# OpenRobotLab/EmbodiedScan

Measured on AMD Instinct MI355X. Metric: scans/sec (train step) mv-3ddet, 20x(480x640) RGB-D views, higher is better.
Workload: dtype bf16; 1 GPU; mv-3ddet ResNet-50(w16) + MinkResNet34 + FCAF3DHeadRotMat, 20 views 480x640, 100k points/scan, bf16 matrix cores with f32 accumulate / f32 master weights, full train step incl. H2D of the batch and AdamW; views=20, parallelism=dp1, h2d=157 MB per step as ONE copy from a pinned slab on a copy stream, double-buffered

## Files before the change

### embodiedscan_amd/csrc/halo.hip

```cpp
#include "common.h"
#include "../../include/es_hip.h"
#include <type_traits>

typedef float f32x4 __attribute__((ext_vector_type(4)));
typedef __bf16 bf16x8_t __attribute__((ext_vector_type(8)));
#ifdef ES_EMU
#define ES_SCHED_FENCE() ((void)0)
#define ES_UNIFORM(x) (x)
#define ES_WAIT_LGKM0() ((void)0)
#else
#define ES_WAIT_LGKM0() __builtin_amdgcn_s_waitcnt(0xC07F)
#define ES_SCHED_FENCE() __builtin_amdgcn_sched_barrier(0)
#define ES_UNIFORM(x) __builtin_amdgcn_readfirstlane(x)
#endif

#define HL_BM 256
#define HL_K 27
#define HL_UMAX 704
#define HL_HT 8192

__device__ __attribute__((aligned(16))) unsigned short g_hl_zero[8];

__global__ __launch_bounds__(512) void k_halo_plan(const int* __restrict__ nbr, int n_out, int K,
                                                   unsigned short* __restrict__ loc, int* __restrict__ hrows,
                                                   int* __restrict__ hcnt) {
  constexpr int NE = HL_BM * HL_K;
  __shared__ __attribute__((aligned(16))) int nb[NE];
  __shared__ unsigned short slotOf[NE];
  __shared__ int hk[HL_HT];
  __shared__ unsigned short hv[HL_HT];
  __shared__ int cnt;
  const int t = threadIdx.x, tile = blockIdx.x;
  const long long e0 = (long long)tile * NE, eN = (long long)n_out * K;
  for (int i = t; i < HL_HT; i += 512) hk[i] = -1;
  if (t == 0) cnt = 0;
  for (int i = t; i < NE / 4; i += 512) {
    int4 v = make_int4(-1, -1, -1, -1);
    const long long e = e0 + (long long)i * 4;
    if (e + 3 < eN) v = *(const int4*)(nbr + e);
    else {
      if (e < eN) v.x = nbr[e];
      if (e + 1 < eN) v.y = nbr[e + 1];
      if (e + 2 < eN) v.z = nbr[e + 2];
    }
    ((int4*)nb)[i] = v;
  }
  __syncthreads();
  for (int e = t; e < NE; e += 512) {
    const int v = nb[e];
    unsigned short so = 0xFFFFu;
    if (v >= 0) {
      unsigned s = ((unsigned)v * 2654435761u) >> (32 - 13);
      for (;;) {
        const int old = atomicCAS(&hk[s], -1, v);
        if (old == -1 || old == v) break;
        s = (s + 1) & (HL_HT - 1);
      }
      so = (unsigned short)s;
    }
    slotOf[e] = so;
  }
  __syncthreads();
  int* const list = nb;
  for (int sl = t; sl < HL_HT; sl += 512) {
    const int v = hk[sl];
    const unsigned long long m = __ballot(v >= 0);
    int base = 0;
    if ((t & 63) == 0 && m) base = atomicAdd(&cnt, __popcll(m));
    base = __shfl(base, 0, 64);
    if (v >= 0) {
      const int pos = base + __popcll(m & ((1ull << (t & 63)) - 1ull));
      list[pos] = v;
      hv[sl] = (unsigned short)pos;
    }
  }
  __syncthreads();
  const int nU = cnt;
  unsigned short* const rk = (unsigned short*)hk;
  int* const hr = hrows + (size_t)tile * NE;
  for (int i = t; i < nU; i += 512) {
    const int v = list[i];
    int r = 0;
    for (int j = 0; j < nU; ++j) r += list[j] < v ? 1 : 0;
    rk[i] = (unsigned short)r;
    hr[r] = v;
  }
  if (t == 0) hcnt[tile] = nU;
  __syncthreads();
  unsigned int* const dst = (unsigned int*)(loc + (size_t)tile * NE);
  for (int i = t; i < NE / 2; i += 512) {
    const unsigned int s0 = slotOf[2 * i], s1 = slotOf[2 * i + 1];
    const unsigned int p0 = s0 == 0xFFFFu ? 0xFFFFu : rk[hv[s0]], p1 = s1 == 0xFFFFu ? 0xFFFFu : rk[hv[s1]];
    dst[i] = p0 | (p1 << 16);
  }
}

extern "C" size_t es_halo_plan_rows(int n_out) { return (size_t)es_cdiv(n_out, HL_BM) * HL_BM; }

extern "C" int es_halo_plan(const int* nbr, int n_out, int K, void* loc, int* hrows, int* hcnt, void* stream) {
  if (n_out <= 0) return 0;
  if (K != HL_K || nbr == nullptr) return -4;
  hipLaunchKernelGGL(k_halo_plan, dim3(es_cdiv(n_out, HL_BM)), dim3(512), 0, (hipStream_t)stream, nbr, n_out, K,
                     (unsigned short*)loc, hrows, hcnt);
  ES_CHECK_LAUNCH();
  return 0;
}

struct HlSeq { int ti, pg, c, tap; };

template <int BNT>
__global__ __launch_bounds__(512, 2) void k_spconv_halo(const unsigned short* __restrict__ Xh, int ldx,
                                                        const unsigned short* __restrict__ W, int Kd, int N,
                                                        const unsigned short* __restrict__ loc, const int* __restrict__ hrows,
                                                        const int* __restrict__ hcnt, int n_out, const float* __restrict__ bias,
                                                        float* __restrict__ Y, int ldy, int accumulate, int colTiles, int total,
                                                        int per, int mirror) {
  constexpr int RB = 128;
  constexpr int ZROW = HL_UMAX;
  constexpr int H_BYTES = (HL_UMAX + 1) * RB;
  constexpr int B_BYTES = BNT * RB;
  constexpr int OFF_B = H_BYTES, OFF_LOC = OFF_B + 3 * B_BYTES, OFF_TAP = OFF_LOC + HL_BM * HL_K * 2;
  constexpr int NH = HL_UMAX * 8 / 512;
  constexpr int NB = BNT / 64;
  constexpr int NF = BNT / 32;
  __shared__ __attribute__((aligned(16))) unsigned char smem[OFF_TAP + 64 * 4];
  unsigned short* const locS = (unsigned short*)(smem + OFF_LOC);
  int* const tapS = (int*)(smem + OFF_TAP);
  const int t = threadIdx.x, lane = t & 63, wv = t >> 6;
  const int wr = wv >> 1, wc = wv & 1;
  for (int it = 0;; ++it) {
  const int lx = (int)(blockIdx.x >> 3) + it * (int)(gridDim.x >> 3);
  const int L = (int)(blockIdx.x & 7) * per + lx;
  if (lx >= per || L >= total) break;
  if (it > 0) __syncthreads();
  const int rt = L / colTiles, ct = L - rt * colTiles;
  const int row0 = rt * HL_BM, n0 = ct * BNT;
  const int nU = hcnt[rt];
  const int nP = nU > HL_UMAX ? (nU + HL_UMAX - 1) / HL_UMAX : 1;
  const int* const hr = hrows + (size_t)rt * HL_BM * HL_K;

  if (t < 32) tapS[t] = 0;
  if (t < 32) ((unsigned int*)(smem + ZROW * RB))[t] = 0u;
  __syncthreads();
  {
    const uint4* g = (const uint4*)(loc + (size_t)row0 * HL_K);
    for (int i = t; i < HL_BM * HL_K / 8; i += 512) {
      const uint4 v = g[i];
      ((uint4*)locS)[i] = v;
      const unsigned int w4[4] = {v.x, v.y, v.z, v.w};
#pragma unroll
      for (int q = 0; q < 8; ++q) {
        const unsigned int p = (w4[q >> 1] >> ((q & 1) * 16)) & 0xFFFFu;
        if (p != 0xFFFFu) tapS[mirror ? HL_K - 1 - (i * 8 + q) % HL_K : (i * 8 + q) % HL_K] = 1;
      }
    }
  }
  __syncthreads();
  unsigned int tm = 0;
  {
    const int f = (lane < HL_K) ? tapS[lane] : 0;
    tm = ES_UNIFORM((unsigned int)__ballot(f));
  }
  const int nT = __popc(tm);

  f32x4 acc[4][NF];
#pragma unroll
  for (int a = 0; a < 4; ++a)
#pragma unroll
    for (int b = 0; b < NF; ++b) acc[a][b] = (f32x4){0.f, 0.f, 0.f, 0.f};

  const int kslot = ((lane & 7) ^ (((wv & 1) * 4 + (lane >> 4)) & 7)) * 8;
  const int b_off0 = (n0 + wv * 8 + (lane >> 3)) * Kd + kslot;
  const int nC = Kd >> 6;
  const int nSteps = nC * nP * nT;
  auto issue_halo = [&](int c0, int page) {
    int h_row[NH];
#pragma unroll
    for (int j = 0; j < NH; ++j) {
      const int u = page * HL_UMAX + (j * 8 + wv) * 8 + (lane >> 3);
      const int r = hr[u < HL_BM * HL_K ? u : HL_BM * HL_K - 1];
      h_row[j] = u < nU ? r : -1;
    }
#pragma unroll
    for (int j = 0; j < NH; ++j) {
      const unsigned short* p = h_row[j] >= 0 ? (Xh + (size_t)h_row[j] * ldx + c0 + kslot) : g_hl_zero;
      __builtin_amdgcn_global_load_lds((const __attribute__((address_space(1))) void*)p,
// ... 54 lines not shown
  if (nSteps > 0) {
    bf16x8_t a0[4], b0[NF], a1[4], b1[NF];
    int idxC[4], rawN[4];
    int s = 0;
    HlSeq q1 = {0, 0, 0, tap_first}, q2 = advance(q1);
    issue_b(0, q1.tap, 0);
    if (nSteps > 1) issue_b(1, q2.tap, q2.c * 64);
    for (int c = 0; c < nC; ++c)
      for (int pg = 0; pg < nP; ++pg) {
        issue_halo(c * 64, pg);
        load_idx(rawN, q1);
        asm volatile("s_waitcnt vmcnt(0)" ::: "memory");
        __syncthreads();
        proc(idxC, rawN, pg);
        read_a(a0, idxC, 0);
        read_b(b0, s % 3, 0);
        q1 = q2; q2 = advance(q2);
        if (nT > 1) load_idx(rawN, q1);
        auto step = [&](auto inner_c) {
          constexpr bool INNER = decltype(inner_c)::value;
          ES_WAIT_LGKM0();
          read_a(a1, idxC, 1);
          read_b(b1, s % 3, 1);
          ES_SCHED_FENCE();
          mma(a0, b0);
          ES_SCHED_FENCE();
          if (INNER || s + 1 < nSteps) {
            asm volatile("s_waitcnt vmcnt(0)" ::: "memory");
            __syncthreads();
            if (s + 2 < nSteps) {
              const HlSeq qn = INNER ? q2 : advance(q1);
              issue_b((s + 2) % 3, qn.tap, qn.c * 64);
            }
          } else {
            ES_WAIT_LGKM0();
          }
          if (INNER) {
            proc(idxC, rawN, pg);
            read_a(a0, idxC, 0);
            read_b(b0, (s + 1) % 3, 0);
            q1 = q2; q2 = advance(q2);
            load_idx(rawN, q1);
          }
          ES_SCHED_FENCE();
          mma(a1, b1);
          ES_SCHED_FENCE();
          ++s;
        };
        for (int ti = 0; ti + 1 < nT; ++ti) step(std::true_type());
        step(std::false_type());
      }
  }
#pragma unroll
  for (int mf = 0; mf < 4; ++mf)
#pragma unroll
    for (int r = 0; r < 4; ++r) {
      const int row = row0 + wr * 64 + mf * 16 + kq * 4 + r;
      if (row < n_out) {
        float* p = Y + (size_t)row * ldy + n0 + wc * (BNT / 2) + li;
        float v[NF];
#pragma unroll
        for (int nf = 0; nf < NF; ++nf) v[nf] = acc[mf][nf][r] + (bias ? bias[n0 + wc * (BNT / 2) + nf * 16 + li] : 0.f);
        if (accumulate) {
          float y0[NF];
#pragma unroll
          for (int nf = 0; nf < NF; ++nf) y0[nf] = p[nf * 16];
#pragma unroll
          for (int nf = 0; nf < NF; ++nf) p[nf * 16] = y0[nf] + v[nf];
        } else {
#pragma unroll
          for (int nf = 0; nf < NF; ++nf) p[nf * 16] = v[nf];
        }
      }
    }
  }
}

static int ES_OPT_HALO_WGS = 0;
static int ES_OPT_HALO_MIN_WGS = 192;

extern "C" int es_halo_set_option(int key, int value) {
  if (key == 30) { ES_OPT_HALO_MIN_WGS = value; return 0; }
  if (key == 31) { ES_OPT_HALO_WGS = value; return 0; }
  return -1;
}

static bool halo_check(int n_in, int ldx, int K, int Cin, int Cout, const void* Xh, const void* W_bf16, const void* loc) {
  if (K != HL_K || (Cin % 64) || (Cout % 128) || (ldx % 8) || ((((uintptr_t)Xh) | ((uintptr_t)W_bf16) | ((uintptr_t)loc)) & 15)) return false;
  return (long long)n_in * ldx < (1ll << 31) && (long long)K * Cout * Cin < (1ll << 31);
}

extern "C" int es_spconv_halo_supported(int n_out, int n_in, int ldx, int K, int Cin, int Cout) {
  if (n_out <= 0 || !halo_check(n_in, ldx, K, Cin, Cout, nullptr, nullptr, nullptr)) return 0;
  return es_cdiv(n_out, HL_BM) * (Cout / 128) >= ES_OPT_HALO_MIN_WGS ? 1 : 0;
}

extern "C" int es_spconv_halo_bf16(const void* Xh, int ldx, const void* W_bf16, const void* loc, const int* hrows, const int* hcnt,
                                   int n_out, int n_in, int K, int Cin, int Cout, const float* bias, float* Y, int ldy,
                                   int accumulate, int mirror, void* stream) {
  if (n_out <= 0) return 0;
  if (!halo_check(n_in, ldx, K, Cin, Cout, Xh, W_bf16, loc)) return -4;
  const int rowTiles = es_cdiv(n_out, HL_BM), colTiles = Cout / 128, total = rowTiles * colTiles, per = es_cdiv(total, 8);
  const int wgs = ES_OPT_HALO_WGS > 0 ? ES_OPT_HALO_WGS : 256;
  hipLaunchKernelGGL((k_spconv_halo<128>), dim3(8 * per < wgs ? 8 * per : (wgs & ~7)), dim3(512), 0, (hipStream_t)stream, (const unsigned short*)Xh, ldx,
                     (const unsigned short*)W_bf16, Cin, Cout, (const unsigned short*)loc, hrows, hcnt, n_out, bias, Y, ldy, accumulate,
                     colTiles, total, per, mirror);
  ES_CHECK_LAUNCH();
  return 0;
}
```

### embodiedscan_amd/csrc/losses.hip

```cpp
#include "common.h"
#include "../../include/es_hip.h"

__global__ __launch_bounds__(256) void k_focal(const float* __restrict__ logits, int ldl,
                                               const int* __restrict__ labels, int N, int C, float gamma,
                                               float alpha, const float* __restrict__ avg_factor, float grad_scale,
                                               float* __restrict__ grad, int ldg, double* __restrict__ partial, int lead, int tail) {
  __shared__ double red[4];
  const float inv = grad_scale / (avg_factor[0] + 1.1920929e-07f);
  const bool g2 = gamma == 2.f;
  const int lane = threadIdx.x & 63;
  double s = 0.0;
  for (int i = blockIdx.x * 4 + (threadIdx.x >> 6); i < N; i += gridDim.x * 4) {
    const int lab = labels[i];
    const float* row = logits + (size_t)i * ldl;
    float* grow = grad ? grad + (size_t)i * ldg : nullptr;
    float acc = 0.f;
    for (int c = lane; c < C; c += 64) {
      float x = row[c];
      float p = 1.f / (1.f + expf(-x));
      float l, g;
      if (lab == c) {
        float q = 1.f - p;
        float lp = logf(fmaxf(p, 1.17549435e-38f));
        float w = g2 ? q * q : powf(q, gamma);
        l = -alpha * w * lp;
        g = -alpha * w * (1.f - p - gamma * p * lp);
      } else {
        float ln = logf(fmaxf(1.f - p, 1.17549435e-38f));
        float w = g2 ? p * p : powf(p, gamma);
        l = -(1.f - alpha) * w * ln;
        g = -(1.f - alpha) * w * (gamma * (1.f - p) * ln - p);
      }
      acc += l;
      if (grow) grow[c] = g * inv;
    }
    if (grow) {
      for (int c = lane; c < lead; c += 64) grow[c - lead] = 0.f;
      for (int c = lane; c < tail; c += 64) grow[C + c] = 0.f;
    }
    s += (double)acc;
  }
  s = es_wave_sum_d(s);
  if (lane == 0) red[threadIdx.x >> 6] = s;
  __syncthreads();
  if (threadIdx.x == 0) partial[blockIdx.x] = red[0] + red[1] + red[2] + red[3];
}
__global__ void k_sum_partials(const double* __restrict__ partial, int n, const float* __restrict__ avg_factor,
                               float* __restrict__ out) {
  __shared__ double red[4];
  double s = 0;
  for (int i = threadIdx.x; i < n; i += blockDim.x) s += partial[i];
  s = es_wave_sum_d(s);
  if ((threadIdx.x & 63) == 0) red[threadIdx.x >> 6] = s;
  __syncthreads();
  if (threadIdx.x == 0) {
    double t = red[0] + red[1] + red[2] + red[3];
    out[0] += avg_factor ? (float)t / (avg_factor[0] + 1.1920929e-07f) : (float)t;
  }
}
#define FOCAL_BLOCKS 2048
extern "C" int es_focal_loss(const float* logits, int ldl, const int* labels, int N, int C, float gamma, float alpha,
                             const float* avg_factor_dev, float grad_scale, float* grad, int ldg, double* partial,
                             float* loss_out, void* stream) {
  return es_focal_loss_clear(logits, ldl, labels, N, C, gamma, alpha, avg_factor_dev, grad_scale, grad, ldg, partial, loss_out, 0, 0,
                             stream);
}
extern "C" int es_focal_loss_clear(const float* logits, int ldl, const int* labels, int N, int C, float gamma, float alpha,
                                   const float* avg_factor_dev, float grad_scale, float* grad, int ldg, double* partial,
                                   float* loss_out, int lead, int tail, void* stream) {
  if (lead < 0 || tail < 0 || ((lead || tail) && (!grad || lead + C + tail > ldg))) return -3;
  hipStream_t st = (hipStream_t)stream;
  int g = es_cdiv(N, 4);
  if (g > FOCAL_BLOCKS) g = FOCAL_BLOCKS;
  if (g < 1) g = 1;
  hipLaunchKernelGGL(k_focal, dim3(g), dim3(256), 0, st, logits, ldl, labels, N, C, gamma, alpha, avg_factor_dev,
                     grad_scale, grad, ldg, partial, lead, tail);
  hipLaunchKernelGGL(k_sum_partials, dim3(1), dim3(256), 0, st, partial, g, avg_factor_dev, loss_out);
  ES_CHECK_LAUNCH();
  return 0;
}

__global__ void k_reg_decode(const float* __restrict__ reg, int ldr, int n, const float* __restrict__ scale,
                             float* __restrict__ bbox) {
  int e = blockIdx.x * blockDim.x + threadIdx.x;
  if (e >= n * 12) return;
  int i = e / 12, c = e - i * 12;
  float v = reg[(size_t)i * ldr + c];
  bbox[e] = c < 6 ? fmaxf(expf(scale[0] * v), 1e-3f) : v;
}
extern "C" int es_reg_decode_fwd(const float* reg, int ldr, int n, const float* scale, float* bbox, void* stream) {
  if (n <= 0) return 0;
  hipLaunchKernelGGL(k_reg_decode, dim3(es_cdiv(n * 12, 256)), dim3(256), 0, (hipStream_t)stream, reg, ldr, n, scale,
                     bbox);
  ES_CHECK_LAUNCH();
  return 0;
}
#define RD_BLOCKS 512
__global__ __launch_bounds__(256) void k_reg_decode_bwd(const float* __restrict__ reg, int ldr, const float* __restrict__ bbox,
                                 const float* __restrict__ dbbox, int n, const float* __restrict__ scale,
                                 float* __restrict__ dreg, int ldg, float* __restrict__ partial) {
  __shared__ float wsum[4];
  float ds = 0.f;
  const size_t tot = (size_t)n * 12;
  for (size_t e = (size_t)blockIdx.x * blockDim.x + threadIdx.x; e < tot; e += (size_t)gridDim.x * blockDim.x) {
    size_t i = e / 12;
    int c = (int)(e - i * 12);
    float g = dbbox[e];
    if (c < 6) {
      float b = bbox[e];
      bool live = b > 1e-3f;
      float gb = live ? g * b : 0.f;
      dreg[i * ldg + c] = gb * scale[0];
      ds += gb * reg[i * ldr + c];
    } else {
      dreg[i * ldg + c] = g;
    }
  }
  ds = es_wave_sum(ds);
  if ((threadIdx.x & 63) == 0) wsum[threadIdx.x >> 6] = ds;
  __syncthreads();
  if (threadIdx.x == 0) partial[blockIdx.x] = ((wsum[0] + wsum[1]) + wsum[2]) + wsum[3];
}
__global__ void k_sum_partials_add(const float* __restrict__ partial, int nb, float* __restrict__ dst) {
  float s = 0.f;
  for (int i = threadIdx.x; i < nb; i += 64) s += partial[i];
  s = es_wave_sum(s);
  if (threadIdx.x == 0) dst[0] += s;
}
extern "C" int es_reg_decode_bwd(const float* reg, int ldr, const float* bbox, const float* dbbox, int n,
                                 const float* scale, float* dreg, int ldg, float* dscale, float* partial, void* stream) {
  if (n <= 0) return 0;
  int g = es_cdiv((long long)n * 12, 256);
  if (g > RD_BLOCKS) g = RD_BLOCKS;
  hipLaunchKernelGGL(k_reg_decode_bwd, dim3(g), dim3(256), 0, (hipStream_t)stream, reg, ldr, bbox, dbbox, n, scale, dreg, ldg,
                     partial);
  hipLaunchKernelGGL(k_sum_partials_add, dim3(1), dim3(64), 0, (hipStream_t)stream, partial, g, dscale);
  ES_CHECK_LAUNCH();
  return 0;
}

typedef double real;
template <int N>
struct Dual {
  real v;
  real d[N];
};
template <int N>
__device__ inline Dual<N> dconst(real v) {
  Dual<N> r; r.v = v;
#pragma unroll
  for (int i = 0; i < N; ++i) r.d[i] = 0;
  return r;
}
template <int N>
__device__ inline Dual<N> dvar(real v, int i) { Dual<N> r = dconst<N>(v); r.d[i] = 1; return r; }
template <int N>
__device__ inline Dual<N> operator+(const Dual<N>& a, const Dual<N>& b) {
  Dual<N> r; r.v = a.v + b.v;
#pragma unroll
// ... 343 lines not shown
```

### embodiedscan_amd/csrc/spconv.hip

```cpp
#include "common.h"
#include "../../include/es_hip.h"

typedef float f32x4 __attribute__((ext_vector_type(4)));

static int ES_OPT_PINGPONG = 1;
static int ES_OPT_WGRAD_HUGE = 1;
static int ES_OPT_ROWGEMM = 1;
static int ES_OPT_WG_BIG_TARGET = 2048;
static int ES_OPT_WG_BIG_ROWS = 512;
static int ES_OPT_WG_SMALL_TARGET = 1024;
static int ES_OPT_WG_CAP_MB = 256;
static int ES_OPT_FWD_SPLIT_WGS = 384;
static int ES_OPT_DMA = 2;
static int ES_OPT_DMA_MIN_CIN = 768;
static int ES_OPT_WGRAD_TR = 1;
static int ES_OPT_ROWGEMM2 = 1;
static int ES_OPT_SPLIT_FOLD = 0;
static int ES_OPT_RG128_MIN_CIN = 0;
static int ES_OPT_NARROW_SLICES = 768;
static int ES_OPT_LIN_SMALL = 256;
static int ES_OPT_EXPAND = 65536;
static int ES_OPT_EXPAND_WGS = 1024;
static int ES_OPT_RG320 = 1;
static int ES_OPT_NARROW = 1;
static int ES_OPT_WSHARE = 0;
static int ES_OPT_RG128_MIN_WGS = 0;
extern int ES_OPT_NORM_CB_ROWS;
extern int ES_OPT_NORM_CB_BWD;
extern int ES_OPT_ELECT_SAFE;
extern int ES_OPT_NORM_CHUNK;
extern "C" int es_set_option(int key, int value) {
  if (key == 1) { ES_OPT_PINGPONG = value; return 0; }
  if (key == 2) { ES_OPT_WGRAD_HUGE = value; return 0; }
  if (key == 3) { ES_OPT_ROWGEMM = value; return 0; }
  if (key == 4) { ES_OPT_WG_BIG_TARGET = value; return 0; }
  if (key == 5) { ES_OPT_WG_BIG_ROWS = value; return 0; }
  if (key == 6) { ES_OPT_WG_SMALL_TARGET = value; return 0; }
  if (key == 7) { ES_OPT_WG_CAP_MB = value; return 0; }
  if (key == 8) { ES_OPT_FWD_SPLIT_WGS = value; return 0; }
  if (key == 9) { ES_OPT_NORM_CHUNK = value; return 0; }
  if (key == 10) { ES_OPT_DMA = value; return 0; }
  if (key == 11) { ES_OPT_DMA_MIN_CIN = value; return 0; }
  if (key == 12) { ES_OPT_RG128_MIN_CIN = value; return 0; }
  if (key == 13) { ES_OPT_ROWGEMM2 = value; return 0; }
  if (key == 14) { ES_OPT_WGRAD_TR = value; return 0; }
  if (key == 15) { ES_OPT_NORM_CB_ROWS = value; return 0; }
  if (key == 16) { ES_OPT_SPLIT_FOLD = value; return 0; }
  if (key == 17) { ES_OPT_NORM_CB_BWD = value; return 0; }
  if (key == 18) { ES_OPT_ELECT_SAFE = value; return 0; }
  if (key == 19) { ES_OPT_RG128_MIN_WGS = value; return 0; }
  if (key == 20) { ES_OPT_WSHARE = value; return 0; }
  if (key == 21) { ES_OPT_NARROW = value; return 0; }
  if (key == 22) { ES_OPT_NARROW_SLICES = value; return 0; }
  if (key == 23) { ES_OPT_RG320 = value; return 0; }
  if (key == 24) { ES_OPT_LIN_SMALL = value; return 0; }
  if (key == 25) { ES_OPT_EXPAND = value; return 0; }
  if (key == 26) { ES_OPT_EXPAND_WGS = value; return 0; }
  return -2;
}


#define BM 128
#define BN 64
#define BK 16
#define LDB (BN + 16)
#define MAXK 27

__device__ inline int a_swz(int row_k) { return (((row_k >> 2) & 3) << 3) ^ ((row_k & 1) << 4); }

template <bool TRANS_W>
__global__ __launch_bounds__(256) void k_spconv(const float* __restrict__ X, int ldx, const float* __restrict__ W,
                                                const int* __restrict__ nbr, int n_out, int n_in, int K, int Cin,
                                                int Cout, const float* __restrict__ bias, float* __restrict__ Y,
                                                int ldy, int accumulate) {
  __shared__ float As[BK * BM];
  __shared__ float Bs[BK * LDB];
  __shared__ int nbrS[BM * MAXK];
  __shared__ int tapAny[32];

  const int t = threadIdx.x, lane = t & 63, wv = t >> 6;
  const int row0 = blockIdx.x * BM, n0 = blockIdx.y * BN;
  const bool vecA = ((ldx & 3) == 0) && ((((uintptr_t)X) & 15) == 0);
  const bool vecB = TRANS_W ? (((Cin & 3) == 0) && ((((uintptr_t)W) & 15) == 0))
                            : (((Cout & 3) == 0) && ((((uintptr_t)W) & 15) == 0));

  if (t < 32) tapAny[t] = 0;
  __syncthreads();
  for (int e = t; e < BM * K; e += 256) {
    int r = e / K, k = e - r * K;
    int j = row0 + r, v = -1;
    if (j < n_out) v = nbr ? nbr[(size_t)j * K + k] : (j < n_in ? j : -1);
    nbrS[e] = v;
    if (v >= 0) tapAny[k] = 1;
  }
  __syncthreads();

  f32x4 acc[2][4];
#pragma unroll
  for (int a = 0; a < 2; ++a)
#pragma unroll
    for (int b = 0; b < 4; ++b) acc[a][b] = (f32x4){0.f, 0.f, 0.f, 0.f};

  const int nC = (Cin + BK - 1) / BK;
  const int a_r = t >> 2, a_kk = (t & 3) * 4;
  const int b_kk = t >> 4, b_n4 = (t & 15) * 4;
  const int bt_n = t >> 2, bt_kk = (t & 3) * 4;

  float ra[2][4], rb[4];
  auto load_chunk = [&](int k, int c0) {
#pragma unroll
    for (int h = 0; h < 2; ++h) {
      int idx = nbrS[(a_r + h * 64) * K + k];
      int c = c0 + a_kk;
      if (idx >= 0 && c < Cin) {
        const float* p = X + (size_t)idx * ldx + c;
        if (vecA && c + 3 < Cin) {
          float4 v = *(const float4*)p;
          ra[h][0] = v.x; ra[h][1] = v.y; ra[h][2] = v.z; ra[h][3] = v.w;
        } else {
#pragma unroll
          for (int e = 0; e < 4; ++e) ra[h][e] = (c + e < Cin) ? p[e] : 0.f;
        }
      } else {
        ra[h][0] = ra[h][1] = ra[h][2] = ra[h][3] = 0.f;
      }
    }
    if (!TRANS_W) {
      int c = c0 + b_kk, n = n0 + b_n4;
      if (c < Cin && n < Cout) {
        const float* p = W + ((size_t)k * Cin + c) * Cout + n;
        if (vecB && n + 3 < Cout) {
          float4 v = *(const float4*)p;
          rb[0] = v.x; rb[1] = v.y; rb[2] = v.z; rb[3] = v.w;
        } else {
#pragma unroll
          for (int e = 0; e < 4; ++e) rb[e] = (n + e < Cout) ? p[e] : 0.f;
        }
      } else {
        rb[0] = rb[1] = rb[2] = rb[3] = 0.f;
      }
    } else {
      int n = n0 + bt_n, c = c0 + bt_kk;
      if (n < Cout && c < Cin) {
        const float* p = W + ((size_t)k * Cout + n) * Cin + c;
        if (vecB && c + 3 < Cin) {
          float4 v = *(const float4*)p;
          rb[0] = v.x; rb[1] = v.y; rb[2] = v.z; rb[3] = v.w;
        } else {
#pragma unroll
          for (int e = 0; e < 4; ++e) rb[e] = (c + e < Cin) ? p[e] : 0.f;
        }
      } else {
        rb[0] = rb[1] = rb[2] = rb[3] = 0.f;
      }
    }
  };
  auto store_chunk = [&]() {
#pragma unroll
    for (int h = 0; h < 2; ++h)
#pragma unroll
      for (int e = 0; e < 4; ++e) {
        int rk = a_kk + e;
        As[rk * BM + ((a_r + h * 64) ^ a_swz(rk))] = ra[h][e];
      }
    if (!TRANS_W) {
      *(float4*)&Bs[b_kk * LDB + b_n4] = make_float4(rb[0], rb[1], rb[2], rb[3]);
    } else {
#pragma unroll
      for (int e = 0; e < 4; ++e) Bs[(bt_kk + e) * LDB + bt_n] = rb[e];
    }
  };

  int k = 0, ci = 0;
  while (k < K && !tapAny[k]) ++k;
  bool have = k < K;
  if (have) load_chunk(k, 0);
  const int li = lane & 15, kq = lane >> 4;
  while (have) {
    store_chunk();
    __syncthreads();
    int nk = k, nci = ci + 1;
    if (nci >= nC) {
      nci = 0;
      ++nk;
      while (nk < K && !tapAny[nk]) ++nk;
    }
    bool nhave = nk < K;
    if (nhave) load_chunk(nk, nci * BK);
#pragma unroll
    for (int ks = 0; ks < BK / 4; ++ks) {
      int rk = ks * 4 + kq;
      int sw = a_swz(rk);
      float a[2], b[4];
#pragma unroll
      for (int mf = 0; mf < 2; ++mf) a[mf] = As[rk * BM + ((wv * 32 + mf * 16 + li) ^ sw)];
#pragma unroll
      for (int nf = 0; nf < 4; ++nf) b[nf] = Bs[rk * LDB + nf * 16 + li];
#pragma unroll
      for (int mf = 0; mf < 2; ++mf)
#pragma unroll
        for (int nf = 0; nf < 4; ++nf)
          acc[mf][nf] = __builtin_amdgcn_mfma_f32_16x16x4f32(a[mf], b[nf], acc[mf][nf], 0, 0, 0);
    }
    __syncthreads();
    k = nk; ci = nci; have = nhave;
  }

#pragma unroll
  for (int mf = 0; mf < 2; ++mf)
#pragma unroll
    for (int nf = 0; nf < 4; ++nf) {
      int col = n0 + nf * 16 + li;
      if (col >= Cout) continue;
      float bv = bias ? bias[col] : 0.f;
#pragma unroll
      for (int r = 0; r < 4; ++r) {
        int row = row0 + wv * 32 + mf * 16 + kq * 4 + r;
        if (row < n_out) {
          float* p = Y + (size_t)row * ldy + col;
          float v = acc[mf][nf][r] + bv;
          *p = accumulate ? (*p + v) : v;
        }
      }
    }
}

#define NW_ROWS 64
#if defined(ES_EMU)
#define NW_UNIFORM(x) (x)
#else
#define NW_UNIFORM(x) __builtin_amdgcn_readfirstlane(x)
#endif
template <int CIN>
__device__ __forceinline__ void narrow_stage(const float* __restrict__ X, int ldx, const int* __restrict__ nbr, int row0,
                                             int n_out, int n_in, float* xg, int* idxS, int* maskS) {
  const int t = threadIdx.x;
  constexpr int NI = (NW_ROWS * 27 + 255) / 256;
  int v[NI];
#pragma unroll
  for (int i = 0; i < NI; ++i) {
    const int e = t + i * 256;
    v[i] = -1;
    if (e < NW_ROWS * 27 && row0 + e / 27 < n_out) v[i] = nbr[(size_t)row0 * 27 + e];
    if (v[i] >= n_in) v[i] = -1;
  }
  float xv[NI][CIN];
#pragma unroll
  for (int i = 0; i < NI; ++i) {
    const float* p = X + (size_t)(v[i] >= 0 ? v[i] : 0) * ldx;
#pragma unroll
    for (int c = 0; c < CIN; ++c) xv[i][c] = p[c];
  }
#pragma unroll
  for (int i = 0; i < NI; ++i) {
    const int e = t + i * 256;
    if (e < NW_ROWS * 27) {
      idxS[e] = v[i];
      const bool ok = v[i] >= 0;
      float4 x4 = make_float4(ok ? xv[i][0] : 0.f, 0.f, 0.f, 0.f);
      if (CIN > 1) x4.y = ok ? xv[i][1] : 0.f;
      if (CIN > 2) x4.z = ok ? xv[i][2] : 0.f;
      if (CIN > 3) x4.w = ok ? xv[i][3] : 0.f;
      *(float4*)&xg[e * 4] = x4;
    }
  }
  __syncthreads();
  if (t < NW_ROWS) {
    int m = 0;
#pragma unroll
    for (int k = 0; k < 27; ++k) m |= (idxS[t * 27 + k] >= 0) ? (1 << k) : 0;
    maskS[t] = m;
  }
  __syncthreads();
}

template <int CIN>
__global__ __launch_bounds__(256) void k_spconv_narrow_fwd(const float* __restrict__ X, int ldx, const float* __restrict__ W,
                                                           const int* __restrict__ nbr, int n_out, int n_in,
                                                           const float* __restrict__ bias, float* __restrict__ Y, int ldy,
                                                           int accumulate) {
  __shared__ __attribute__((aligned(16))) float xg[NW_ROWS * 27 * 4];
  __shared__ int idxS[NW_ROWS * 27];
  __shared__ int maskS[NW_ROWS];
  const int t = threadIdx.x, co = t & 63, wv = t >> 6;
  float w[27][CIN];
#pragma unroll
  for (int k = 0; k < 27; ++k)
#pragma unroll
    for (int c = 0; c < CIN; ++c) w[k][c] = W[(k * CIN + c) * 64 + co];
  const float bv = bias ? bias[co] : 0.f;
  const int tiles = (n_out + NW_ROWS - 1) / NW_ROWS;
  for (int tile = blockIdx.x; tile < tiles; tile += gridDim.x) {
    const int row0 = tile * NW_ROWS;
    narrow_stage<CIN>(X, ldx, nbr, row0, n_out, n_in, xg, idxS, maskS);
    for (int rr = 0; rr < NW_ROWS / 4; ++rr) {
      const int r = wv * (NW_ROWS / 4) + rr;
      if (row0 + r >= n_out) break;
      const int m = NW_UNIFORM(maskS[r]);
      float acc = bv;
#pragma unroll
      for (int k = 0; k < 27; ++k)
        if (m & (1 << k)) {
          const float4 x4 = *(const float4*)&xg[(r * 27 + k) * 4];
          acc = fmaf(x4.x, w[k][0], acc);
          if (CIN > 1) acc = fmaf(x4.y, w[k][1], acc);
          if (CIN > 2) acc = fmaf(x4.z, w[k][2], acc);
          if (CIN > 3) acc = fmaf(x4.w, w[k][3], acc);
        }
      float* p = Y + (size_t)(row0 + r) * ldy + co;
      *p = accumulate ? (*p + acc) : acc;
    }
    __syncthreads();
  }
}
static bool narrow_ok(const int* nbr, int K, int Cin, int Cout) { return ES_OPT_NARROW && nbr != nullptr && K == 27 && Cin == 3 && Cout == 64; }

extern "C" int es_spconv_fwd(const float* X, int ldx, const float* W, const int* nbr, int n_out, int n_in, int K,
                             int Cin, int Cout, const float* bias, float* Y, int ldy, int trans_w, int accumulate,
                             void* stream) {
  if (n_out <= 0 || Cout <= 0) return 0;
  if (K > MAXK) return -2;
  if (!trans_w && narrow_ok(nbr, K, Cin, Cout)) {
    const int tiles = es_cdiv(n_out, NW_ROWS);
    hipLaunchKernelGGL(k_spconv_narrow_fwd<3>, dim3(tiles > 2048 ? 2048 : tiles), dim3(256), 0, (hipStream_t)stream, X, ldx, W, nbr,
                       n_out, n_in, bias, Y, ldy, accumulate);
    ES_CHECK_LAUNCH();
    return 0;
  }
  dim3 grid(es_cdiv(n_out, BM), es_cdiv(Cout, BN));
  if (trans_w)
    hipLaunchKernelGGL(k_spconv<true>, grid, dim3(256), 0, (hipStream_t)stream, X, ldx, W, nbr, n_out, n_in, K, Cin,
                       Cout, bias, Y, ldy, accumulate);
  else
    hipLaunchKernelGGL(k_spconv<false>, grid, dim3(256), 0, (hipStream_t)stream, X, ldx, W, nbr, n_out, n_in, K,
                       Cin, Cout, bias, Y, ldy, accumulate);
  ES_CHECK_LAUNCH();
  return 0;
}

__device__ __forceinline__ void wgrad_emit(float* __restrict__ dW, float* __restrict__ ws, int bz, size_t dw_floats,
                                           size_t off, float v, int accumulate) {
  if (ws) ws[(size_t)bz * dw_floats + off] = v;
  else if (accumulate) dW[off] += v;
  else dW[off] = v;
}
#define WM 64
#define WN 64
#define WR 16
#define LDW (64 + 16)
__global__ __launch_bounds__(256) void k_spconv_wgrad(const float* __restrict__ X, int ldx,
                                                      const float* __restrict__ dY, int ldy,
                                                      const int* __restrict__ nbr, int n_out, int n_in, int K,
                                                      int Cin, int Cout, int rows_per_split,
                                                      float* __restrict__ dW, float* __restrict__ ws, int accumulate) {
  __shared__ float As[WR * LDW];
  __shared__ float Bs[WR * LDW];
  const int t = threadIdx.x, lane = t & 63, wv = t >> 6;
  const int nCt = (Cin + WM - 1) / WM;
  const int k = blockIdx.x / nCt, c0 = (blockIdx.x % nCt) * WM;
  const int n0 = blockIdx.y * WN;
  const int rbeg = blockIdx.z * rows_per_split;
  const int rend = min(n_out, rbeg + rows_per_split);
  const bool vecA = ((ldx & 3) == 0) && ((((uintptr_t)X) & 15) == 0);
  const bool vecB = ((ldy & 3) == 0) && ((((uintptr_t)dY) & 15) == 0);
  const int lr = t >> 4, l4 = (t & 15) * 4;
  const int li = lane & 15, kq = lane >> 4;

  f32x4 acc[4];
#pragma unroll
  for (int b = 0; b < 4; ++b) acc[b] = (f32x4){0.f, 0.f, 0.f, 0.f};

  float ra[4], rb[4];
  auto load_rows = [&](int r0) {
    int j = r0 + lr;
    int idx = -1;
    if (j < rend) idx = nbr ? nbr[(size_t)j * K + k] : (j < n_in ? j : -1);
    int c = c0 + l4, n = n0 + l4;
    if (idx >= 0 && c < Cin) {
      const float* p = X + (size_t)idx * ldx + c;
      if (vecA && c + 3 < Cin) {
        float4 v = *(const float4*)p;
        ra[0] = v.x; ra[1] = v.y; ra[2] = v.z; ra[3] = v.w;
      } else {
#pragma unroll
        for (int e = 0; e < 4; ++e) ra[e] = (c + e < Cin) ? p[e] : 0.f;
      }
    } else {
      ra[0] = ra[1] = ra[2] = ra[3] = 0.f;
    }
    if (idx >= 0 && n < Cout) {
      const float* p = dY + (size_t)j * ldy + n;
      if (vecB && n + 3 < Cout) {
        float4 v = *(const float4*)p;
        rb[0] = v.x; rb[1] = v.y; rb[2] = v.z; rb[3] = v.w;
      } else {
#pragma unroll
        for (int e = 0; e < 4; ++e) rb[e] = (n + e < Cout) ? p[e] : 0.f;
      }
    } else {
      rb[0] = rb[1] = rb[2] = rb[3] = 0.f;
    }
  };

  if (rbeg < rend) load_rows(rbeg);
// ... 112 lines not shown
    for (int z = 1; z < splits; ++z) s += ws[(size_t)z * n + e];
    dW[e] = accumulate ? dW[e] + s : s;
  }
}
__global__ void k_wgrad_reduce4(const float4* __restrict__ ws, int splits, size_t n4, float4* __restrict__ dW, int accumulate) {
  for (size_t e = (size_t)blockIdx.x * blockDim.x + threadIdx.x; e < n4; e += (size_t)gridDim.x * blockDim.x) {
    float4 s = ws[e];
    for (int z = 1; z < splits; ++z) {
      float4 v = ws[(size_t)z * n4 + e];
      s.x += v.x; s.y += v.y; s.z += v.z; s.w += v.w;
    }
    if (accumulate) {
      float4 d = dW[e];
      s = make_float4(d.x + s.x, d.y + s.y, d.z + s.z, d.w + s.w);
    }
    dW[e] = s;
  }
}
template <int R>
__global__ __launch_bounds__(256) void k_wgrad_reduce_ranges(const float* __restrict__ ws, int splits, size_t n,
                                                             float* __restrict__ dW, int accumulate) {
  constexpr int EB = 256 / R;
  __shared__ float part[R][EB];
  const int el = threadIdx.x % EB, rr = threadIdx.x / EB;
  const size_t e = (size_t)blockIdx.x * EB + el;
  const int per = (splits + R - 1) / R;
  const int z0 = rr * per, z1 = min(splits, z0 + per);
  float s = 0.f;
  if (e < n)
    for (int z = z0; z < z1; ++z) s += ws[(size_t)z * n + e];
  part[rr][el] = s;
  __syncthreads();
  if (rr == 0 && e < n) {
    float t = part[0][el];
#pragma unroll
    for (int r = 1; r < R; ++r) t += part[r][el];
    dW[e] = accumulate ? dW[e] + t : t;
  }
}
static int wgrad_reduce(const float* ws, int splits, size_t n, float* dW, int accumulate, hipStream_t st) {
  if (splits <= 1 || n == 0) return 0;
  if (splits >= 64) {
    if (splits >= 512) hipLaunchKernelGGL(k_wgrad_reduce_ranges<64>, dim3(es_cdiv((long long)n, 4)), dim3(256), 0, st, ws, splits, n, dW, accumulate);
    else hipLaunchKernelGGL(k_wgrad_reduce_ranges<16>, dim3(es_cdiv((long long)n, 16)), dim3(256), 0, st, ws, splits, n, dW, accumulate);
  } else if ((n % 4 == 0) && (((((uintptr_t)ws) | ((uintptr_t)dW)) & 15) == 0)) {
    int g = es_cdiv((long long)(n / 4), 256);
    hipLaunchKernelGGL(k_wgrad_reduce4, dim3(g > 8192 ? 8192 : g), dim3(256), 0, st, (const float4*)ws, splits, n / 4, (float4*)dW, accumulate);
  } else {
    int g = es_cdiv((long long)n, 256);
    hipLaunchKernelGGL(k_wgrad_reduce, dim3(g > 8192 ? 8192 : g), dim3(256), 0, st, ws, splits, n, dW, accumulate);
  }
  ES_CHECK_LAUNCH();
  return 0;
}

extern "C" int es_spconv_wgrad(const float* X, int ldx, const float* dY, int ldy, const int* nbr, int n_out,
                               int n_in, int K, int Cin, int Cout, float* dW, int accumulate, float* ws, size_t ws_floats,
                               void* stream) {
  if (n_out <= 0 || Cin <= 0 || Cout <= 0) return 0;
  WgradPlan p = wgrad_plan_f32(n_out, K, Cin, Cout, ws != nullptr);
  const size_t nw = (size_t)K * Cin * Cout;
  if (p.splits > 1 && ws_floats < (size_t)p.splits * nw) return -5;
  if (p.kind == 4 && nbr != nullptr) {
    hipLaunchKernelGGL(k_spconv_narrow_wgrad<3>, dim3(p.splits), dim3(256), 0, (hipStream_t)stream, X, ldx, dY, ldy, nbr, n_out, n_in,
                       p.rows_per_split, dW, p.splits > 1 ? ws : nullptr, accumulate);
    ES_CHECK_LAUNCH();
    return wgrad_reduce(ws, p.splits, nw, dW, accumulate, (hipStream_t)stream);
  }
  dim3 grid(K * es_cdiv(Cin, WM), es_cdiv(Cout, WN), p.splits);
  hipLaunchKernelGGL(k_spconv_wgrad, grid, dim3(256), 0, (hipStream_t)stream, X, ldx, dY, ldy, nbr, n_out, n_in, K,
                     Cin, Cout, p.rows_per_split, dW, p.splits > 1 ? ws : nullptr, accumulate);
  ES_CHECK_LAUNCH();
  return wgrad_reduce(ws, p.splits, nw, dW, accumulate, (hipStream_t)stream);
}

typedef __bf16 bf16x2_t __attribute__((ext_vector_type(2)));
typedef __bf16 bf16x8_t __attribute__((ext_vector_type(8)));
typedef float f32x2_t __attribute__((ext_vector_type(2)));
#define HBK 32
#define HLD (HBK + 16)

#define ES_IO_Y16 1
#define ES_IO_R16 2
#define ES_IO_WSHARE 0x10000
__device__ __forceinline__ float4 bf16x4_to_f32(uint2 v) {
  return make_float4(__uint_as_float(v.x << 16), __uint_as_float(v.x & 0xffff0000u), __uint_as_float(v.y << 16),
                     __uint_as_float(v.y & 0xffff0000u));
}
__device__ __forceinline__ float ep_activate(float v, int act) {
  return act == 2 ? (v > 0.f ? v : expf(v) - 1.f) : fmaxf(v, 0.f);
}
__device__ inline uint32_t pack_bf16(float a, float b) {
  f32x2_t x = {a, b};
  bf16x2_t y = __builtin_convertvector(x, bf16x2_t);
  return *(uint32_t*)&y;
}

template <int BNT>
__global__ __launch_bounds__(256) void k_spconv_bf16(const float* __restrict__ X, int ldx,
                                                     const unsigned short* __restrict__ W ,
                                                     const int* __restrict__ nbr, int n_out, int n_in, int K, int Cin,
                                                     int Cout, const float* __restrict__ bias, float* __restrict__ Y,
                                                     int ldy, int accumulate,
                                                     const float* __restrict__ ep_scale,
                                                     const float* __restrict__ ep_shift,
                                                     const float* __restrict__ ep_res, int ep_ldr, int ep_act, int x_half,
                                                     int io) {
  constexpr int NF = BNT / 16;
  constexpr int NB = BNT / 64;
  __shared__ __attribute__((aligned(16))) unsigned short As[BM * HLD];
  __shared__ __attribute__((aligned(16))) unsigned short Bs[BNT * HLD];
  __shared__ int nbrS[BM * MAXK];
  __shared__ int tapAny[32];
  const int t = threadIdx.x, lane = t & 63, wv = t >> 6;
  const int row0 = blockIdx.x * BM, n0 = blockIdx.y * BNT;
  const bool vecA = ((ldx & 3) == 0) && ((((uintptr_t)X) & 15) == 0);
  const bool vecB = ((Cin & 7) == 0) && ((((uintptr_t)W) & 15) == 0);

  if (t < 32) tapAny[t] = 0;
  __syncthreads();
  for (int e = t; e < BM * K; e += 256) {
    int r = e / K, k = e - r * K;
    int j = row0 + r, v = -1;
    if (j < n_out) v = nbr ? nbr[(size_t)j * K + k] : (j < n_in ? j : -1);
    nbrS[e] = v;
    if (v >= 0) tapAny[k] = 1;
  }
  __syncthreads();

  f32x4 acc[2][NF];
#pragma unroll
  for (int a = 0; a < 2; ++a)
#pragma unroll
    for (int b = 0; b < NF; ++b) acc[a][b] = (f32x4){0.f, 0.f, 0.f, 0.f};

  const int nC = (Cin + HBK - 1) / HBK;
  const int a_r = t >> 1, a_kk = (t & 1) * 16;
  const int b_n = t >> 2, b_kk = (t & 3) * 8;
  struct Regs { float4 a[4]; uint4 b[NB]; };
  struct It { int k, ci; };

  auto load_chunk = [&](Regs& R, It it) {
    int c0 = it.ci * HBK;
    int idx = nbrS[a_r * K + it.k];
    int c = c0 + a_kk;
    if (idx >= 0 && c < Cin && x_half) {
      const unsigned short* ph = (const unsigned short*)X + (size_t)idx * ldx + c;
      if (c + 15 < Cin && (ldx & 7) == 0 && ((((uintptr_t)X) & 15) == 0)) {
        const uint4 u0 = ((const uint4*)ph)[0], u1 = ((const uint4*)ph)[1];
        R.a[0] = make_float4(__uint_as_float(u0.x << 16), __uint_as_float(u0.x & 0xffff0000u), __uint_as_float(u0.y << 16),
                             __uint_as_float(u0.y & 0xffff0000u));
        R.a[1] = make_float4(__uint_as_float(u0.z << 16), __uint_as_float(u0.z & 0xffff0000u), __uint_as_float(u0.w << 16),
                             __uint_as_float(u0.w & 0xffff0000u));
        R.a[2] = make_float4(__uint_as_float(u1.x << 16), __uint_as_float(u1.x & 0xffff0000u), __uint_as_float(u1.y << 16),
                             __uint_as_float(u1.y & 0xffff0000u));
        R.a[3] = make_float4(__uint_as_float(u1.z << 16), __uint_as_float(u1.z & 0xffff0000u), __uint_as_float(u1.w << 16),
                             __uint_as_float(u1.w & 0xffff0000u));
      } else {
        float v[16];
#pragma unroll
        for (int q = 0; q < 16; ++q) v[q] = (c + q < Cin) ? __uint_as_float((uint32_t)ph[q] << 16) : 0.f;
#pragma unroll
        for (int q = 0; q < 4; ++q) R.a[q] = make_float4(v[4 * q], v[4 * q + 1], v[4 * q + 2], v[4 * q + 3]);
      }
    } else if (idx >= 0 && c < Cin) {
      const float* p = X + (size_t)idx * ldx + c;
      if (vecA && c + 15 < Cin) {
#pragma unroll
        for (int q = 0; q < 4; ++q) R.a[q] = ((const float4*)p)[q];
      } else {
        float v[16];
#pragma unroll
        for (int q = 0; q < 16; ++q) v[q] = (c + q < Cin) ? p[q] : 0.f;
#pragma unroll
        for (int q = 0; q < 4; ++q) R.a[q] = make_float4(v[4 * q], v[4 * q + 1], v[4 * q + 2], v[4 * q + 3]);
      }
    } else {
#pragma unroll
      for (int q = 0; q < 4; ++q) R.a[q] = make_float4(0.f, 0.f, 0.f, 0.f);
    }
#pragma unroll
    for (int h = 0; h < NB; ++h) {
      int n = n0 + b_n + h * 64, cb = c0 + b_kk;
      if (n < Cout && cb < Cin) {
        const unsigned short* p = W + ((size_t)it.k * Cout + n) * Cin + cb;
        if (vecB && cb + 7 < Cin) {
          R.b[h] = *(const uint4*)p;
        } else {
          unsigned short hh[8];
#pragma unroll
          for (int q = 0; q < 8; ++q) hh[q] = (cb + q < Cin) ? p[q] : (unsigned short)0;
          R.b[h].x = hh[0] | ((uint32_t)hh[1] << 16); R.b[h].y = hh[2] | ((uint32_t)hh[3] << 16);
          R.b[h].z = hh[4] | ((uint32_t)hh[5] << 16); R.b[h].w = hh[6] | ((uint32_t)hh[7] << 16);
        }
      } else {
        R.b[h] = make_uint4(0u, 0u, 0u, 0u);
      }
    }
  };
  auto store_chunk = [&](const Regs& R) {
    uint4* pa = (uint4*)&As[a_r * HLD + a_kk];
    pa[0] = make_uint4(pack_bf16(R.a[0].x, R.a[0].y), pack_bf16(R.a[0].z, R.a[0].w), pack_bf16(R.a[1].x, R.a[1].y),
                       pack_bf16(R.a[1].z, R.a[1].w));
    pa[1] = make_uint4(pack_bf16(R.a[2].x, R.a[2].y), pack_bf16(R.a[2].z, R.a[2].w), pack_bf16(R.a[3].x, R.a[3].y),
                       pack_bf16(R.a[3].z, R.a[3].w));
#pragma unroll
    for (int h = 0; h < NB; ++h) *(uint4*)&Bs[(b_n + h * 64) * HLD + b_kk] = R.b[h];
// ... 70 lines not shown
          } else {
            if (ep_res) v += rv;
            if (ep_act) v = ep_activate(v, ep_act);
          }
          if (io & ES_IO_Y16) {
            float vn = __shfl_xor(v, 1, 64);
            if (!(li & 1)) *(uint32_t*)((unsigned short*)Y + (size_t)row * ldy + col) = pack_bf16(v, vn);
          } else {
            *p = accumulate ? (*p + v) : v;
          }
        }
      }
    }
}

#define ES_SPLIT_TICKETS 1024
template <int BNT_>
__device__ inline void split_tail(const float* ws, unsigned int* tickets, int row0, int n0, int n_out, int Cout,
                                  float* __restrict__ Y, int ldy, int accumulate) {
  if (!es_last_block_release_only(tickets + blockIdx.y * gridDim.x + blockIdx.x, gridDim.z)) return;
  const int split = gridDim.z;
  constexpr int C4 = BNT_ / 4;
  const size_t tot = (size_t)n_out * Cout;
  const bool vec = ((ldy & 3) == 0) && ((((uintptr_t)Y) & 15) == 0);
  for (int e = threadIdx.x; e < BM * C4; e += blockDim.x) {
    const int row = row0 + e / C4, col = n0 + (e % C4) * 4;
    if (row >= n_out) break;
    const float* p0 = ws + (size_t)row * Cout + col;
    float4 sum = *(const float4*)p0;
    for (int z = 1; z < split; ++z) {
      float4 v = *(const float4*)(p0 + (size_t)z * tot);
      sum.x += v.x; sum.y += v.y; sum.z += v.z; sum.w += v.w;
    }
    float* y = Y + (size_t)row * ldy + col;
    if (vec) {
      if (accumulate) { float4 y0 = *(const float4*)y; sum.x = y0.x + sum.x; sum.y = y0.y + sum.y; sum.z = y0.z + sum.z; sum.w = y0.w + sum.w; }
      *(float4*)y = sum;
    } else {
      y[0] = accumulate ? y[0] + sum.x : sum.x; y[1] = accumulate ? y[1] + sum.y : sum.y;
      y[2] = accumulate ? y[2] + sum.z : sum.z; y[3] = accumulate ? y[3] + sum.w : sum.w;
    }
  }
}

template <int BNT, bool XH, bool PP>
__global__ __launch_bounds__(256, 3) void k_spconv_bf16_fast(const void* __restrict__ Xv, int ldx,
                                                          const unsigned short* __restrict__ W,
                                                          const int* __restrict__ nbr, int n_out, int n_in, int K,
                                                          int Cin, int Cout, const float* __restrict__ bias,
                                                          float* __restrict__ Y, int ldy, int accumulate,
                                                          const float* __restrict__ ep_scale,
                                                          const float* __restrict__ ep_shift,
                                                          const float* __restrict__ ep_res, int ep_ldr, int ep_act, int io) {
  constexpr int NF = BNT / 16;
  constexpr int NB = BNT / 64;
  constexpr int NBUF = PP ? 2 : 1;
  constexpr int LDP = PP ? HBK : HLD;
  __shared__ __attribute__((aligned(16))) unsigned short As[NBUF * BM * LDP];
  __shared__ __attribute__((aligned(16))) unsigned short Bs[NBUF * BNT * LDP];
  __shared__ int nbrS[BM * MAXK];
  __shared__ int taps[32];
  __shared__ int nTaps;
  const int t = threadIdx.x, lane = t & 63, wv = t >> 6;
  int bx = blockIdx.x, by = blockIdx.y, bz = blockIdx.z;
  if (io & ES_IO_WSHARE) {
    const int gx = gridDim.x, gy = gridDim.y, L = bx + gx * (by + gy * bz);
    const int full = ((gy * (int)gridDim.z) >> 3) << 3;
    if (L < full * gx) {
      const int j = L >> 3, pair = (j / gx) * 8 + (L & 7);
      bx = j % gx; by = pair % gy; bz = pair / gy;
    }
  }
  const int row0 = bx * BM, n0 = by * BNT;

  __shared__ int tapFlag[32];
  if (t < 32) tapFlag[t] = 0;
  __syncthreads();
  {
    int r = t >> 1, kh = (K + 1) >> 1, k0 = (t & 1) * kh, k1 = min(K, k0 + kh);
    int j = row0 + r;
    const int* src = nbr ? nbr + (size_t)j * K : nullptr;
    for (int k = k0; k < k1; ++k) {
      int v = -1;
      if (j < n_out) v = src ? src[k] : (j < n_in ? j : -1);
      nbrS[r * K + k] = v;
      if (v >= 0) tapFlag[k] = 1;
    }
  }
  __syncthreads();
  if (t < 64) {
    int f = (t < K) ? tapFlag[t] : 0;
    unsigned long long m = __ballot(f);
    if (f) taps[__popcll(m & ((1ull << t) - 1ull))] = t;
    if (t == 0) nTaps = __popcll(m);
  }
  __syncthreads();
  const int nTall = nTaps;
  const int tBeg = (int)(((long long)nTall * bz) / gridDim.z);
  const int nT = (int)(((long long)nTall * (bz + 1)) / gridDim.z);

  f32x4 acc[2][NF];
#pragma unroll
  for (int a = 0; a < 2; ++a)
#pragma unroll
    for (int b = 0; b < NF; ++b) acc[a][b] = (f32x4){0.f, 0.f, 0.f, 0.f};

  const int nC = Cin / HBK;
  const int a_r = t >> 1, a_kk = (t & 1) * 16;
  const int b_n = t >> 2, b_kk = (t & 3) * 8;
  const int b_row = (n0 + b_n) * Cin + b_kk;
  const int w_tap = Cout * Cin;
  const float* X = (const float*)Xv;
  const unsigned short* Xh = (const unsigned short*)Xv;
  struct Regs { float4 a[XH ? 2 : 4]; uint4 b[NB]; int valid; };
  struct It { int ti, ci, a_off, b_off, valid; };
  auto set_tap = [&](It& it) {
    int ti = it.ti < nT ? it.ti : (nT - 1);
    int k = taps[ti];
    int idx = nbrS[a_r * K + k];
    it.valid = (idx >= 0) && (it.ti < nT);
    it.a_off = (idx >= 0 ? idx : 0) * ldx + a_kk;
    it.b_off = k * w_tap + b_row;
  };
  auto advance = [&](It& it) {
    if (++it.ci >= nC) {
      it.ci = 0;
      ++it.ti;
      set_tap(it);
    }
  };
  auto load_chunk = [&](Regs& R, const It& it) {
    int c0 = it.ci * HBK;
    if (XH) {
      const float4* p = (const float4*)(Xh + it.a_off + c0);
      R.a[0] = p[0];
      R.a[1] = p[1];
    } else {
      const float4* p = (const float4*)(X + it.a_off + c0);
#pragma unroll
      for (int q = 0; q < (XH ? 2 : 4); ++q) R.a[q] = p[q];
    }
#pragma unroll
    for (int h = 0; h < NB; ++h) R.b[h] = *(const uint4*)(W + it.b_off + h * 64 * Cin + c0);
    R.valid = it.valid;
  };
  const int a_sw = PP ? (((a_r >> 2) * 3) & 3) : 0, b_sw = PP ? (((b_n >> 2) * 3) & 3) : 0;
  auto store_chunk = [&](const Regs& R, int buf = 0) {
    uint4* pa = (uint4*)&As[buf * BM * LDP + a_r * LDP + (PP ? 0 : a_kk)];
    uint4 v0, v1;
    if (XH) {
      v0 = make_uint4(__float_as_uint(R.a[0].x), __float_as_uint(R.a[0].y), __float_as_uint(R.a[0].z),
                      __float_as_uint(R.a[0].w));
      v1 = make_uint4(__float_as_uint(R.a[1].x), __float_as_uint(R.a[1].y), __float_as_uint(R.a[1].z),
                      __float_as_uint(R.a[1].w));
    } else {
      constexpr int H = XH ? 0 : 2;
      v0 = make_uint4(pack_bf16(R.a[0].x, R.a[0].y), pack_bf16(R.a[0].z, R.a[0].w), pack_bf16(R.a[1].x, R.a[1].y),
                      pack_bf16(R.a[1].z, R.a[1].w));
      v1 = make_uint4(pack_bf16(R.a[H].x, R.a[H].y), pack_bf16(R.a[H].z, R.a[H].w), pack_bf16(R.a[H + 1].x, R.a[H + 1].y),
                      pack_bf16(R.a[H + 1].z, R.a[H + 1].w));
    }
    if (!R.valid) v0 = v1 = make_uint4(0u, 0u, 0u, 0u);
    if (PP) {
      const int g0 = (t & 1) * 2;
      pa[(g0 ^ a_sw)] = v0;
      pa[((g0 + 1) ^ a_sw)] = v1;
#pragma unroll
// ... 66 lines not shown
        advance(i1);
        load_chunk(r1, i1);
        compute();
        __syncthreads();
      }
    }
  }
#pragma unroll
  for (int mf = 0; mf < 2; ++mf)
#pragma unroll
    for (int nf = 0; nf < NF; ++nf) {
      int col = n0 + nf * 16 + li;
      float bv = bias ? bias[col] : 0.f;
      float sc = ep_scale ? ep_scale[col] : 1.f, sh = (ep_shift && gridDim.z == 1) ? ep_shift[col] : 0.f;
#pragma unroll
      for (int r = 0; r < 4; ++r) {
        int row = row0 + wv * 32 + mf * 16 + kq * 4 + r;
        if (row < n_out) {
          float* p = Y + (size_t)row * ldy + col;
          if (gridDim.z > 1) {
            float v = acc[mf][nf][r] + (bz == 0 ? bv : 0.f);
            const_cast<float*>(ep_res)[((size_t)bz * n_out + row) * Cout + col] = v;
          } else {
            float v = acc[mf][nf][r] + bv;
            if (ep_scale) v = v * sc + sh;
            float rv = 0.f;
            if (ep_res) {
              if (io & ES_IO_R16) rv = __uint_as_float((uint32_t)((const unsigned short*)ep_res)[(size_t)row * ep_ldr + col] << 16);
              else rv = ep_res[(size_t)row * ep_ldr + col];
            }
            if (ep_act == 3) {
              if (!(rv > 0.f)) v = 0.f;
            } else {
              if (ep_res) v += rv;
              if (ep_act) v = ep_activate(v, ep_act);
            }
            if (io & ES_IO_Y16) {
              float vn = __shfl_xor(v, 1, 64);
              if (!(li & 1)) *(uint32_t*)((unsigned short*)Y + (size_t)row * ldy + col) = pack_bf16(v, vn);
            } else {
              *p = accumulate ? (*p + v) : v;
            }
          }
        }
      }
    }
  if (gridDim.z > 1 && ep_shift) split_tail<BNT>(ep_res, (unsigned int*)ep_shift, row0, n0, n_out, Cout, Y, ldy, accumulate);
}

__device__ __attribute__((aligned(16))) unsigned short g_zero_granule[8];

template <int BNT, int KB, int NBUF = 2>
__global__ __launch_bounds__(256, (KB == 1 && NBUF == 2) ? 3 : 2) void k_spconv_bf16_dma(
    const unsigned short* __restrict__ Xh, int ldx, const unsigned short* __restrict__ W, const int* __restrict__ nbr,
    int n_out, int n_in, int K, int Cin, int Cout, const float* __restrict__ bias, float* __restrict__ Y, int ldy,
    int accumulate, const float* __restrict__ ep_scale, const float* __restrict__ ep_shift,
    const float* __restrict__ ep_res, int ep_ldr, int ep_act, int io) {
  constexpr int G = 4 * KB;
  constexpr int RB = 64 * KB;
  constexpr int BKT = 32 * KB;
  constexpr int A_BYTES = BM * RB, B_BYTES = BNT * RB;
  constexpr int NA = BM * G / 256, NBI = BNT * G / 256;
  constexpr int NFW = BNT / 32;
  constexpr int OFF_B = NBUF * A_BYTES, OFF_MAP = OFF_B + NBUF * B_BYTES, OFF_TAPS = OFF_MAP + BM * MAXK * 4,
                OFF_FLAG = OFF_TAPS + 32 * 4, OFF_NT = OFF_FLAG + 32 * 4;
  __shared__ __attribute__((aligned(16))) unsigned char smem[OFF_NT + 16];
  int* const nbrS = (int*)(smem + OFF_MAP);
  int* const taps = (int*)(smem + OFF_TAPS);
  int* const tapFlag = (int*)(smem + OFF_FLAG);
  int* const nTapsP = (int*)(smem + OFF_NT);
  const int t = threadIdx.x, lane = t & 63, wv = t >> 6;
  const int wr = wv >> 1, wc = wv & 1;
  const int bz = blockIdx.z;
  const int row0 = blockIdx.x * BM, n0 = blockIdx.y * BNT;

  if (t < 32) tapFlag[t] = 0;
  __syncthreads();
  {
    int r = t >> 1, kh = (K + 1) >> 1, k0 = (t & 1) * kh, k1 = min(K, k0 + kh);
    int j = row0 + r;
    const int* src = nbr ? nbr + (size_t)j * K : nullptr;
    for (int k = k0; k < k1; ++k) {
      int v = -1;
      if (j < n_out) v = src ? src[k] : (j < n_in ? j : -1);
      nbrS[r * K + k] = v;
      if (v >= 0) tapFlag[k] = 1;
    }
  }
  __syncthreads();
  if (t < 64) {
    int f = (t < K) ? tapFlag[t] : 0;
    unsigned long long m = __ballot(f);
    if (f) taps[__popcll(m & ((1ull << t) - 1ull))] = t;
    if (t == 0) *nTapsP = __popcll(m);
  }
  __syncthreads();
  const int nTall = *nTapsP;
  const int tBeg = (int)(((long long)nTall * bz) / gridDim.z);
  const int nT = (int)(((long long)nTall * (bz + 1)) / gridDim.z);

  f32x4 acc[4][NFW];
#pragma unroll
  for (int a = 0; a < 4; ++a)
#pragma unroll
    for (int b = 0; b < NFW; ++b) acc[a][b] = (f32x4){0.f, 0.f, 0.f, 0.f};

  auto key = [](int row) { return KB == 1 ? (((row >> 2) * 3) & 3) : ((row >> 1) & 7); };
  int a_row[NA], a_g8[NA], b_off[NBI];
#pragma unroll
  for (int j = 0; j < NA; ++j) {
    int e = (j * 4 + wv) * 64 + lane, row = e / G, slot = e % G;
    a_row[j] = row;
    a_g8[j] = (slot ^ key(row)) * 8;
  }
#pragma unroll
  for (int j = 0; j < NBI; ++j) {
    int e = (j * 4 + wv) * 64 + lane, row = e / G, slot = e % G;
    b_off[j] = (n0 + row) * Cin + (slot ^ key(row)) * 8;
  }
  const int nC = Cin / BKT;
  const int w_tap = Cout * Cin;
  int it_ti = tBeg, it_c0 = 0, tap_off = 0;
  int a_off[NA];
  auto set_tap = [&]() {
    int k = taps[it_ti < nT ? it_ti : (nT - 1)];
    tap_off = k * w_tap;
#pragma unroll
    for (int j = 0; j < NA; ++j) {
      int idx = nbrS[a_row[j] * K + k];
      a_off[j] = idx >= 0 ? idx * ldx + a_g8[j] : -1;
    }
  };
  auto issue = [&](int buf) {
#pragma unroll
    for (int j = 0; j < NA; ++j) {
      const unsigned short* p = a_off[j] >= 0 ? (Xh + a_off[j] + it_c0) : g_zero_granule;
      __builtin_amdgcn_global_load_lds((const __attribute__((address_space(1))) void*)p,
                                       (__attribute__((address_space(3))) void*)(smem + buf * A_BYTES + (j * 4 + wv) * 1024),
                                       16, 0, 0);
    }
#pragma unroll
    for (int j = 0; j < NBI; ++j) {
      const unsigned short* p = W + tap_off + b_off[j] + it_c0;
      __builtin_amdgcn_global_load_lds((const __attribute__((address_space(1))) void*)p,
                                       (__attribute__((address_space(3))) void*)(smem + OFF_B + buf * B_BYTES + (j * 4 + wv) * 1024),
                                       16, 0, 0);
    }
    it_c0 += BKT;
    if (it_c0 >= Cin) {
      it_c0 = 0;
      ++it_ti;
      set_tap();
    }
  };
  const int li = lane & 15, kq = lane >> 4;
  const int f_key = key(li);
  const unsigned char* a_frag = smem + (wr * 64 + li) * RB;
  const unsigned char* b_frag = smem + OFF_B + (wc * (BNT / 2) + li) * RB;
  auto compute = [&](int buf) {
#pragma unroll
    for (int h = 0; h < KB; ++h) {
      const int so = ((h * 4 + kq) ^ f_key) * 16;
      bf16x8_t a[4], b[NFW];
#pragma unroll
      for (int mf = 0; mf < 4; ++mf) a[mf] = *(const bf16x8_t*)(a_frag + buf * A_BYTES + mf * 16 * RB + so);
#pragma unroll
      for (int nf = 0; nf < NFW; ++nf) b[nf] = *(const bf16x8_t*)(b_frag + buf * B_BYTES + nf * 16 * RB + so);
// ... 524 lines not shown
    const int ks_n = min(LS_KS, Cin - k0 + 31 & ~31) / 32;
    for (int ks = 0; ks < ks_n; ++ks) {
      const bf16x8_t a = *(const bf16x8_t*)&As[(wv * 16 + li) * LS_LD + ks * 32 + kq * 8];
#pragma unroll
      for (int nf = 0; nf < 4; ++nf) {
        const bf16x8_t b = *(const bf16x8_t*)&Bs[(32 * (nf >> 1) + 4 * (nf & 1) + wrow) * LS_LD + ks * 32 + kq * 8];
        acc[nf] = __builtin_amdgcn_mfma_f32_16x16x32_bf16(b, a, acc[nf], 0, 0, 0);
      }
    }
    __syncthreads();
  }
  const int row = row0 + wv * 16 + li;
  if (row < n) {
#pragma unroll
    for (int p2 = 0; p2 < 2; ++p2) {
      const int col = n0 + 32 * p2 + kq * 8;
      float o[8];
#pragma unroll
      for (int r = 0; r < 4; ++r) { o[r] = acc[2 * p2][r]; o[4 + r] = acc[2 * p2 + 1][r]; }
      if (bias) {
        const float4 b0 = *(const float4*)(bias + col), b1 = *(const float4*)(bias + col + 4);
        o[0] += b0.x; o[1] += b0.y; o[2] += b0.z; o[3] += b0.w; o[4] += b1.x; o[5] += b1.y; o[6] += b1.z; o[7] += b1.w;
      }
      float4* py = (float4*)(Y + (size_t)row * ldy + col);
      if (accumulate) {
        const float4 y0 = py[0], y1 = py[1];
        o[0] += y0.x; o[1] += y0.y; o[2] += y0.z; o[3] += y0.w; o[4] += y1.x; o[5] += y1.y; o[6] += y1.z; o[7] += y1.w;
      }
      py[0] = make_float4(o[0], o[1], o[2], o[3]);
      py[1] = make_float4(o[4], o[5], o[6], o[7]);
    }
  }
}

extern "C" int es_spconv_bf16_is_fast(int n_in, int ldx, int K, int Cin, int Cout) {
  return (Cin % HBK == 0) && (ldx % 8 == 0) && (Cout % 64 == 0) && ((long long)n_in * ldx < (1ll << 31)) &&
         ((long long)K * Cout * Cin < (1ll << 31));
}

static int split_factor(int n_out, int K, int Cout) {
  int wgs = (Cout % 128 == 0) ? es_cdiv(n_out, BM) * (Cout / 128) : es_cdiv(n_out, BM) * (Cout / 64);
  int split = 1;
  while (split < 8 && wgs * split < ES_OPT_FWD_SPLIT_WGS && split * 3 <= K) split *= 2;
  return split;
}
__global__ void k_sum_splits(const float* __restrict__ ws, int split, int n_out, int Cout, float* __restrict__ Y, int ldy,
                             int accumulate) {
  size_t tot = (size_t)n_out * Cout;
  for (size_t e = (size_t)blockIdx.x * blockDim.x + threadIdx.x; e < tot; e += (size_t)gridDim.x * blockDim.x) {
    float s = ws[e];
    for (int z = 1; z < split; ++z) s += ws[(size_t)z * tot + e];
    size_t row = e / Cout;
    float* p = Y + row * ldy + (e - row * Cout);
    *p = accumulate ? (*p + s) : s;
  }
}
__global__ void k_sum_splits4(const float4* __restrict__ ws, int split, size_t tot4, int C4, float* __restrict__ Y, int ldy,
                              int accumulate) {
  for (size_t e = (size_t)blockIdx.x * blockDim.x + threadIdx.x; e < tot4; e += (size_t)gridDim.x * blockDim.x) {
    float4 s = ws[e];
    for (int z = 1; z < split; ++z) {
      float4 v = ws[(size_t)z * tot4 + e];
      s.x += v.x; s.y += v.y; s.z += v.z; s.w += v.w;
    }
    size_t row = e / C4;
    float4* p = (float4*)(Y + row * ldy + (e - row * C4) * 4);
    if (accumulate) { float4 y0 = *p; s.x = y0.x + s.x; s.y = y0.y + s.y; s.z = y0.z + s.z; s.w = y0.w + s.w; }
    *p = s;
  }
}
extern "C" size_t es_spconv_split_workspace_floats(int n_out, int K, int Cin, int Cout) {
  if (K <= 1 || Cin % HBK != 0 || Cout % 64 != 0 || n_out <= 0) return 0;
  int split = split_factor(n_out, K, Cout);
  return split > 1 ? (size_t)ES_SPLIT_TICKETS + (size_t)split * n_out * Cout : 0;
}

static int spconv_fwd_bf16_impl(const void* Xv, int x_is_bf16, int ldx, const void* W_bf16, const int* nbr, int n_out,
                                int n_in, int K, int Cin, int Cout, const float* bias, float* Y, int ldy,
                                int accumulate, const float* ep_scale, const float* ep_shift, const float* ep_res,
                                int ep_ldr, int ep_act, void* stream, float* ws = nullptr, size_t ws_floats = 0,
                                int y_half = 0, int r_half = 0) {
  if (n_out <= 0 || Cout <= 0) return 0;
  if (K > MAXK) return -2;
  int io = (y_half ? ES_IO_Y16 : 0) | ((r_half && ep_res) ? ES_IO_R16 : 0) | (y_half & 0xff00);
  if (y_half && (accumulate || (ldy % 4) || (Cout % 4) || (((uintptr_t)Y) & 7))) return -7;
  if ((io & ES_IO_R16) && ((ep_ldr % 4) || (((uintptr_t)ep_res) & 7))) return -7;
  hipStream_t st = (hipStream_t)stream;
  const unsigned short* Wh = (const unsigned short*)W_bf16;
  const float* X = (const float*)Xv;
  bool fast = (Cin % HBK == 0) && (ldx % (x_is_bf16 ? 8 : 4) == 0) && ((((uintptr_t)Xv) & 15) == 0) &&
              ((((uintptr_t)Wh) & 15) == 0) && ((long long)n_in * ldx < (1ll << 31)) &&
              ((long long)K * Cout * Cin < (1ll << 31)) && (Cout % 64 == 0);
  dim3 g128(es_cdiv(n_out, BM), Cout / 128), g64(es_cdiv(n_out, BM), Cout / 64);
  if (ES_OPT_ROWGEMM && K == 1 && nbr == nullptr && ep_act != 7 && n_in >= n_out && (Cin % 8 == 0) &&
      (Cout % 16 == 0) && (ldx % (x_is_bf16 ? 8 : 4) == 0) && (ldy % 4 == 0) &&
      (((((uintptr_t)Xv) | ((uintptr_t)Wh)) & 15) == 0) && ((((uintptr_t)Y) & (y_half ? 7 : 15)) == 0) &&
      (!ep_res || ((ep_ldr % 4 == 0) && ((((uintptr_t)ep_res) & ((io & ES_IO_R16) ? 7 : 15)) == 0)))) {
    const bool wide = Cout % 128 == 0 && Cin >= ES_OPT_RG128_MIN_CIN &&
                      (long long)es_cdiv(n_out, BM) * (Cout / 128) >= ES_OPT_RG128_MIN_WGS;
    if (ES_OPT_EXPAND && x_is_bf16 && y_half && !(y_half & 0xff00) && ep_scale && ep_shift && !bias && !accumulate && (ep_act == 0 || ep_act == 1) &&
        (!ep_res || r_half) && Cout == 4 * Cin && (Cin == 16 || Cin == 32 || Cin == 64) && n_out >= ES_OPT_EXPAND && n_in >= n_out &&
        (ldx % 8 == 0) && (ldy % 8 == 0) && (!ep_res || (ep_ldr % 8 == 0 && ((((uintptr_t)ep_res) & 15) == 0))) && ((((uintptr_t)Y) & 15) == 0) &&
        (((((uintptr_t)ep_scale) | ((uintptr_t)ep_shift)) & 15) == 0) && (long long)n_out * (ldy > ldx ? ldy : ldx) < (1ll << 31)) {
      const int rt = 4 / (Cout / 64), tiles = es_cdiv(n_out, 16), want = es_cdiv(tiles, rt);
      dim3 ge(want < ES_OPT_EXPAND_WGS ? want : ES_OPT_EXPAND_WGS);
#define EX_LAUNCH(C_) hipLaunchKernelGGL((k_expand_bf16<C_>), ge, dim3(256), 0, st, (const unsigned short*)Xv, ldx, Wh, n_out, ep_scale, ep_shift, \
                                         (const unsigned short*)ep_res, ep_ldr, ep_act, (unsigned short*)Y, ldy)
      if (Cin == 16) EX_LAUNCH(16);
      else if (Cin == 32) EX_LAUNCH(32);
      else EX_LAUNCH(64);
#undef EX_LAUNCH
      ES_CHECK_LAUNCH();
      return 0;
    }
    if (ES_OPT_LIN_SMALL && !x_is_bf16 && !y_half && !ep_scale && !ep_res && !ep_act && (Cin % 8 == 0) && (Cout % 64 == 0) && Cin >= 64 &&
        (long long)es_cdiv(n_out, BM) * es_cdiv(Cout, 128) < ES_OPT_LIN_SMALL && n_in >= n_out && (ldy % 4 == 0) && ((((uintptr_t)Y) & 15) == 0) &&
        (!bias || ((((uintptr_t)bias) & 15) == 0))) {
      hipLaunchKernelGGL(k_lin_small, dim3(es_cdiv(n_out, 64), Cout / 64), dim3(256), 0, st, X, ldx, Wh, n_out, Cin, Cout, bias, Y, ldy, accumulate);
      ES_CHECK_LAUNCH();
      return 0;
    }
    const bool whole = ES_OPT_RG320 && Cout == 320 && n_out >= 16384 && !ep_res && !accumulate && !y_half && ES_OPT_ROWGEMM2 && (ldy % 4 == 0) && ((((uintptr_t)Y) & 15) == 0);
    const int nt = whole ? 320 : wide ? 128 : (Cout % 64 == 0) ? 64 : (Cout % 32 == 0) ? 32 : 16;
    dim3 g(es_cdiv(n_out, BM), Cout / nt);
#define RG_LAUNCH(NT_)                                                                                              \
    do {                                                                                                            \
      if (x_is_bf16)                                                                                                \
        hipLaunchKernelGGL((k_rowgemm_bf16<NT_, true>), g, dim3(256), 0, st, Xv, ldx, Wh, n_out, n_in, Cin, Cout, bias, Y, ldy, \
                           accumulate, ep_scale, ep_shift, ep_res, ep_ldr, ep_act, io);                              \
      else                                                                                                          \
        hipLaunchKernelGGL((k_rowgemm_bf16<NT_, false>), g, dim3(256), 0, st, Xv, ldx, Wh, n_out, n_in, Cin, Cout, bias, Y, ldy, \
                           accumulate, ep_scale, ep_shift, ep_res, ep_ldr, ep_act, io);                              \
    } while (0)
#define RG2_LAUNCH(NT_)                                                                                             \
    do {                                                                                                            \
      if (x_is_bf16)                                                                                                \
        hipLaunchKernelGGL((k_rowgemm2_bf16<NT_, true>), g, dim3(256), 0, st, Xv, ldx, Wh, n_out, n_in, Cin, Cout, bias, Y, ldy, \
                           accumulate, ep_scale, ep_shift, ep_res, ep_ldr, ep_act, io, RowGemmTaps{0, 0, 1, 0, 0});   \
      else                                                                                                          \
        hipLaunchKernelGGL((k_rowgemm2_bf16<NT_, false>), g, dim3(256), 0, st, Xv, ldx, Wh, n_out, n_in, Cin, Cout, bias, Y, ldy, \
                           accumulate, ep_scale, ep_shift, ep_res, ep_ldr, ep_act, io, RowGemmTaps{0, 0, 1, 0, 0});  \
    } while (0)
    const bool g2 = ES_OPT_ROWGEMM2 && nt >= 32 && (ldy % (y_half ? 8 : 4) == 0) && ((((uintptr_t)Y) & 15) == 0) &&
                    (!ep_res || ((ep_ldr % ((io & ES_IO_R16) ? 8 : 4) == 0) && ((((uintptr_t)ep_res) & 15) == 0)));
    if (whole) {
      if (x_is_bf16)
        hipLaunchKernelGGL((k_rowgemm2_bf16<320, true, false, false>), g, dim3(256), 0, st, Xv, ldx, Wh, n_out, n_in, Cin, Cout, bias, Y, ldy,
                           0, ep_scale, ep_shift, (const float*)nullptr, 0, ep_act, io, RowGemmTaps{0, 0, 1, 0, 0});
      else
        hipLaunchKernelGGL((k_rowgemm2_bf16<320, false, false, false>), g, dim3(256), 0, st, Xv, ldx, Wh, n_out, n_in, Cin, Cout, bias, Y, ldy,
                           0, ep_scale, ep_shift, (const float*)nullptr, 0, ep_act, io, RowGemmTaps{0, 0, 1, 0, 0});
    } else if (g2 && nt == 128) RG2_LAUNCH(128);
    else if (g2 && nt == 64) RG2_LAUNCH(64);
    else if (g2) RG2_LAUNCH(32);
    else if (nt == 128) RG_LAUNCH(128);
    else if (nt == 64) RG_LAUNCH(64);
    else if (nt == 32) RG_LAUNCH(32);
    else RG_LAUNCH(16);
#undef RG2_LAUNCH
#undef RG_LAUNCH
    ES_CHECK_LAUNCH();
    return 0;
  }
  int det_split = 0;
  if (fast && !(ep_scale || ep_res || ep_act) && K > 1 && !y_half) {
    int split = split_factor(n_out, K, Cout);
    const int tiles = (Cout % 128 == 0) ? g128.x * g128.y : g64.x * g64.y;
// ... 915 lines not shown
```

### embodiedscan_amd/engine.py

```python
import os

import torch
from . import hip
from .hip import P, call, iarr


def _stream():
    return hip.stream()


_NEW_VARS = None


class Var:
    __slots__ = ('d', 'g', 'rg', 'dh', 'gh', 'gate', 'gated', 'fresh')

    def __init__(self, d, rg=True):
        self.d, self.g, self.rg = d, None, rg
        self.dh = self.gh = None
        if _NEW_VARS is not None:
            _NEW_VARS.append(self)
        self.fresh = False
        self.gate = None
        self.gated = False
# ... 365 lines not shown
            ws[:min(ws.numel(), 2048)].zero_()


def drop_caches():
    for table in _WS.values():
        table.clear()
    _KEEP.clear()


MARKS = None


HOST_MARKS = None


def mark(name):
    if HOST_MARKS is not None:
        import time
        HOST_MARKS.append((name, time.perf_counter()))
    if MARKS is not None:
        ev = torch.cuda.Event(enable_timing=True)
        ev.record(hip.stream_obj())
        MARKS.append((name, ev))


DEBUG_GRADS = None
DEBUG_CONV = None
DEBUG_OPS = None
DEBUG_FWD = None


def fwd_record(kind, entry, **ops):
    rec = dict(kind=kind, entry=entry, precision=PRECISION[0])
    for k, v in ops.items():
        if isinstance(v, (Param, ParamSlice)):
            rec[k] = v.d.clone()
            if PRECISION[0] == 'bf16' and v.d.dim() == 3:
                rec[k + '_h'] = v.bf16()[1].clone()
        elif isinstance(v, torch.Tensor):
            rec[k] = v.clone()
        else:
            rec[k] = v
    if callable(DEBUG_FWD):
        DEBUG_FWD(rec)
    else:
        DEBUG_FWD.append(rec)


def _cast_rows(t):
    n, C = t.shape
    h = torch.empty((n, C), dtype=torch.bfloat16, device=t.device)
    call('es_cast_rows_bf16', P(t), t.stride(0), n, C, P(h), _stream())
    return h


GEN_FUSED = [os.environ.get('ES_GEN_FUSED', '1') != '0']


def _split_ws(n_out, K, cin, cout, like):
    if K <= 1 or n_out <= 0:
        return None, 0
    nf = int(hip.raw('es_spconv_split_workspace_floats')(n_out, K, cin, cout))
    if nf == 0:
        return None, 0
    return ticket_ws(nf, like, tag='split')


def _fwd_bf16(X, x_is_bf16, ldx, Wp, nbr, n_out, n_in, K, cin, cout, bias_p, Y, ldy, acc, like):
    ws, nf = _split_ws(n_out, K, cin, cout, like)
    if ws is not None:
        call('es_spconv_fwd_bf16_ws', X, x_is_bf16, ldx, Wp, nbr, n_out, n_in, K, cin, cout, bias_p, Y, ldy, acc, P(ws), nf, _stream())
        return 'es_spconv_fwd_bf16_ws'
    call('es_spconv_fwd_bf16', X, x_is_bf16, ldx, Wp, nbr, n_out, n_in, K, cin, cout, bias_p, Y, ldy, acc, _stream())
    return 'es_spconv_fwd_bf16'


def _use_shadow(n_rows, C, K, cin, cout):
    return K > 1 and hip.raw('es_spconv_bf16_is_fast')(n_rows, C, K, cin, cout) == 1


HALO = [os.environ.get('ES_HALO', '1') != '0']
if os.environ.get('ES_HALO_MIN_WGS') is not None:
    hip.raw('es_halo_set_option')(30, int(os.environ['ES_HALO_MIN_WGS']))


def _halo_ok(nbr, n_out, n_in, ldx, K, cin, cout):
    return (HALO[0] and K == 27 and nbr is not None
            and hip.raw('es_spconv_halo_supported')(n_out, n_in, ldx, K, cin, cout) == 1)


def halo_plan(nbr):
    plan = getattr(nbr, '_halo', None)
    if plan is None:
        n_out, K = nbr.shape
        rows = int(hip.raw('es_halo_plan_rows')(n_out))
        loc = torch.empty((rows, K), dtype=torch.int16, device=nbr.device)
        hrows = torch.empty((rows // 256, 256 * K), dtype=torch.int32, device=nbr.device)
        hcnt = torch.empty((rows // 256,), dtype=torch.int32, device=nbr.device)
        call('es_halo_plan', P(nbr), n_out, K, P(loc), P(hrows), P(hcnt), _stream())
        plan = nbr._halo = (loc, hrows, hcnt)
        if hip.PROFILE is not None:
            hip.PAIRS[loc.data_ptr()] = (nbr >= 0).sum()
    return plan


def _halo_launch(Xh, ldx, Wp, nbr, n_out, n_in, K, cin, cout, bias_p, Y, ldy, acc):
    fwd = getattr(nbr, '_mirror_of', None)
    loc, hrows, hcnt = halo_plan(fwd if fwd is not None else nbr)
    return hip.try_call('es_spconv_halo_bf16', Xh, ldx, Wp, P(loc), P(hrows), P(hcnt), n_out, n_in, K, cin, cout, bias_p, Y, ldy, acc,
                        int(fwd is not None), _stream())


def empty(shape, like, dtype=torch.float32):
    return torch.empty(shape, dtype=dtype, device=like.device)


def zeros(shape, like, dtype=torch.float32):
    return torch.zeros(shape, dtype=dtype, device=like.device)


def _ld(t):
    assert t.dim() == 2 and t.stride(1) == 1, 'row matrices must be contiguous along channels'
    return t.stride(0)


def _grad_target(v, shape_like):
    v.gh = None
    if v.g is None:
        v.g = torch.empty(shape_like.shape, dtype=torch.float32, device=shape_like.device)
        return v.g, 0
    return v.g, 1



DENSE = [os.environ.get('ES_DENSE', '1') != '0']


def _dense_geom(dense):
    return iarr(dense) if dense is not None else None


def dense_ok(dense, mode, cin, cout):
    if not (DENSE[0] and dense is not None and PRECISION[0] == 'bf16'):
        return False
    if mode == 2 and dense[4] == 1 and (cin // 256) * (cout // 256) < 48:
        return False
    return hip.raw('es_dconv_supported')(_dense_geom(dense), mode, cin, cout) == 1


def _dense_launch(Xh, ldx, Wp, dense, mode, cin, cout, Y, ldy, acc, like):
    g = _dense_geom(dense)
    s = _stream()
    need = int(hip.raw('es_dconv_workspace_floats')(g, mode, cin, cout))
    ws, nf = stream_ws(s, 'dense', need, like) if need else (None, 0)
    return hip.try_call('es_dconv_fwd_bf16', Xh, ldx, Wp, g, mode, cin, cout, Y, ldy, acc, P(ws), nf, s)


def _dense_wgrad(xh, ldx, gh, ldy, dense, transposed, cin, cout, dW, acc, sw, like):
    g = _dense_geom(dense)
    need = int(hip.raw('es_dconv_wgrad_workspace_floats')(g, transposed, cin, cout))
    ws, nf = stream_ws(sw, 'dense', need, like) if need else (None, 0)
    return hip.try_call('es_dconv_wgrad_ws_bf16', xh, ldx, gh, ldy, g, transposed, cin, cout, dW, acc, P(ws), nf, sw)


class _Maps:
    __slots__ = ('fn', 'val')

    def __init__(self, fn):
        self.fn, self.val = fn, None

    def get(self):
        if self.val is None:
            self.val = self.fn()
        return self.val


def conv(x, w, nbr, inv, n_out, bias=None, need_dx=True, bias_from=0, dense=None, maps=None):
    K, cin, cout = w.d.shape
    n_in = x.d.shape[0]
    y = Var(empty((n_out, cout), x.d))
    bf = PRECISION[0] == 'bf16' and cin >= 16
    if maps is not None:
        maps = _Maps(maps) if not isinstance(maps, _Maps) else maps
    x16 = x.d.dtype == torch.bfloat16
    if x16:
        assert bf and _ld(x.d) == cin, 'bf16 input rows need the bf16 kernels and contiguous rows'
        x.dh = x.d
    dn = bf and _ld(x.d) == cin and dense_ok(dense, 0, cin, cout)
    if dn and bias:
        y.d.copy_(bias.d.expand_as(y.d))
# ... 41 lines not shown
def _conv_backward(x, w, nbr, inv, n_out, y, gy, bias, bias_from, need_dx, bf, gate=None, dense=None, maps=None, img=None):
    K, cin, cout = w.d.shape
    rec = None
    dn_ok = bf and dense is not None and gate is None and _ld(gy) == cout and _ld(x.d) == cin
    dn_w = dense if (dn_ok and w.g is not None and dense_ok(dense, 2, cin, cout)) else None
    dn_d = dense if (dn_ok and need_dx and x.rg and dense_ok(dense, 1, cin, cout)) else None
    if maps is not None and (DEBUG_CONV is not None or (w.g is not None and dn_w is None) or (need_dx and x.rg and dn_d is None)):
        nbr, inv = maps.get()
    if DEBUG_CONV is not None:
        rec = dict(x=x.d, w=w, nbr=nbr, n_out=n_out, gy=gy.clone(), bf=bool(bf), gate=gate, need_dx=bool(need_dx and x.rg),
                   before=(x.g.clone() if (x.g is not None and need_dx and x.rg) else None), bias=bias, bias_from=bias_from)
        DEBUG_CONV.append(rec)
    gh = None
    if dn_w is not None or dn_d is not None or (
            bf and cout >= 16 and need_dx and x.rg and gate is None and _ld(gy) == cout and _use_shadow(n_out, cout, K, cout, cin)):
        gh = y.grad_shadow() if gy is y.g else _cast_rows(gy)
    if dn_w is not None:
        x.shadow()
    if w.g is not None or (bias is not None and bias.g is not None):
        sw = _wgrad_stream(gy, x.d, gh, x.dh)
    if w.g is not None:
        _conv_wgrad(x, w, nbr, n_out, gy, gh, bf, dn_w, maps, img, sw)
    if bias is not None and bias.g is not None:
        nb, dst = cout - bias_from, bias.g.data_ptr() + 4 * bias_from
        ws, nf = stream_ws(sw, 'colsum', int(hip.raw('es_colsum_workspace_floats')(n_out, nb)), gy)
        call('es_colsum', gy.data_ptr() + 4 * bias_from, _ld(gy), n_out, nb, dst, _first_write(dst), P(ws), nf, sw)
    if need_dx and x.rg:
        _conv_dgrad(x, w, inv, n_out, gy, gh, bf, dn_d, maps, gate, img)
    if rec is not None and rec['need_dx']:
        rec['after'] = x.g.clone()


def _conv_wgrad(x, w, nbr, n_out, gy, gh, bf, dn_w, maps, img, sw):
    K, cin, cout = w.d.shape
    n_in = x.d.shape[0]
    acc = _first_write(P(w.g))
    xh_f32 = bf and x.dh is not None and gy.dtype == torch.float32
    if dn_w is not None:
        if _dense_wgrad(P(x.dh), cin, P(gh), cout, dn_w, 0, cin, cout, P(w.g), acc, sw, gh):
            return
        if maps is not None:
            nbr, _ = maps.get()
            sw = _wgrad_stream()
    if IMG_WGRAD[0] and xh_f32 and img is not None and K == 9 and cin == cout:
        nf = int(hip.raw('es_img_wgrad9_workspace_floats')(img[0], img[1], img[2], cin, img[3]))
        if nf:
            ws, nf = stream_ws(sw, 'wgrad', nf, gy)
            if hip.try_call('es_img_wgrad9_bf16', P(x.dh), _ld(x.dh), P(gy), _ld(gy), img[0], img[1], img[2], cin, img[3], P(w.g), acc,
                            P(ws), nf, sw):
                return
    if xh_f32 and K == 1 and nbr is None and n_in == n_out:
        nf = int(hip.raw('es_rows_wgrad1_workspace_floats')(n_out, cin, cout))
        if nf:
            ws, nf = stream_ws(sw, 'wgrad', nf, gy)
            if hip.try_call('es_rows_wgrad1_bf16', P(x.dh), _ld(x.dh), P(gy), _ld(gy), n_out, cin, cout, P(w.g), acc, P(ws), nf, sw):
                return
    if bf and (gh is not None or x.dh is not None or x.d.dtype == torch.bfloat16):
        xs, ys = x.dh if x.dh is not None else x.d, gh if gh is not None else gy
        _wgrad('es_spconv_wgrad_bf16_src', sw, P(w.g), P(xs), int(x.dh is not None), _ld(xs), P(ys), int(gh is not None), _ld(ys),
               P(nbr), n_out, n_in, K, cin, cout, like=gy, acc=acc)
        return
    assert x.d.dtype == torch.float32, 'bf16 activation rows reach the weight gradient through their shadow (x.dh)'
    _wgrad('es_spconv_wgrad_bf16' if bf else 'es_spconv_wgrad', sw, P(w.g), P(x.d), _ld(x.d), P(gy), _ld(gy), P(nbr), n_out, n_in, K,
           cin, cout, like=gy, acc=acc)


def _conv_dgrad(x, w, inv, n_out, gy, gh, bf, dn_d, maps, gate, img):
    K, cin, cout = w.d.shape
    n_in = x.d.shape[0]
    s = _stream()
    if gate is not None:
        assert x.g is None and bf, 'gated dgrad: x must have exactly one consumer'
        x.g, x.gated = torch.empty(x.d.shape, dtype=torch.float32, device=x.d.device), True
        if (img is not None and K == 9 and img[3] == 1 and cin == cout and x.d.dtype == torch.bfloat16 and gy.dtype == torch.float32
                and _ld(x.d) == cin and hip.raw('es_img_conv3_supported')(img[0], img[1], img[2], cin, 1, 1) == 1
                and hip.try_call('es_img_conv3_bf16', P(gy), _ld(gy), P(w.bf16()[0]), img[0], img[1], img[2], cin, 1, 1, P(gate), 0, P(x.d),
                                 _ld(x.d), 3, P(x.g), 0, _ld(x.g), s)):
            return
        if (IMG_STRIDED_DGRAD[0] and img is not None and K == 9 and img[3] == 2 and cin == cout and x.d.dtype == torch.bfloat16
                and gy.dtype == torch.float32 and hip.raw('es_img_dgrad3_s2_supported')(img[0], img[1], img[2], cin) == 1
                and hip.try_call('es_img_dgrad3_s2_bf16', P(gy), _ld(gy), P(w.bf16()[0]), img[0], img[1], img[2], cin, P(gate), P(x.d),
                                 _ld(x.d), P(x.g), _ld(x.g), s)):
            return
        if x.d.dtype == torch.bfloat16:
            call('es_spconv_fwd_bf16_io', P(gy), 0, _ld(gy), P(w.bf16()[0]), P(inv), n_in, n_out, K, cout, cin, P(gate), 0,
                 P(x.d), 1, _ld(x.d), 3, P(x.g), 0, _ld(x.g), s)
        else:
            call('es_spconv_fwd_bf16_affine', P(gy), _ld(gy), P(w.bf16()[0]), P(inv), n_in, n_out, K, cout, cin, P(gate), 0,
                 P(x.d), _ld(x.d), 3, P(x.g), _ld(x.g), s)
        return
    g, acc = _grad_target(x, x.d)
    if (IMG_STRIDED_DGRAD[0] and img is not None and K == 1 and img[3] == 2 and bf and gh is None and dn_d is None
            and gy.dtype == torch.float32 and g.dtype == torch.float32 and n_in == img[0] * img[1] * img[2]
            and hip.raw('es_img_dgrad1_s2_supported')(img[0], img[1], img[2], cout, cin) == 1
            and hip.try_call('es_img_dgrad1_s2_bf16', P(gy), _ld(gy), P(w.bf16()[0]), img[0], img[1], img[2], cout, cin, P(g), _ld(g), acc, s)):
        return
    if dn_d is not None:
        if _dense_launch(P(gh), cout, P(w.bf16()[0]), dn_d, 1, cin, cout, P(g), _ld(g), acc, gh):
            return
        if maps is not None:
            _, inv = maps.get()
    if gh is not None and _halo_ok(inv, n_in, n_out, cout, K, cout, cin) and \
            _halo_launch(P(gh), cout, P(w.bf16()[0]), inv, n_in, n_out, K, cout, cin, 0, P(g), _ld(g), acc):
        return
    if gh is not None:
        _fwd_bf16(P(gh), 1, cout, P(w.bf16()[0]), P(inv), n_in, n_out, K, cout, cin, 0, P(g), _ld(g), acc, gh)
    elif bf and cout >= 16:
        _fwd_bf16(P(gy), 0, _ld(gy), P(w.bf16()[0]), P(inv), n_in, n_out, K, cout, cin, 0, P(g), _ld(g), acc, gy)
    else:
        call('es_spconv_fwd', P(gy), _ld(gy), P(w.d), P(inv), n_in, n_out, K, cout, cin, 0, P(g), _ld(g), 1, acc, s)


def conv_affine(x, w, nbr, inv, n_out, scale, shift, act=1, res=None, need_dx=True, sole_consumer=False, out_bf16=False, img=None):
    K, cin, cout = w.d.shape
    n_in = x.d.shape[0]
    if PRECISION[0] != 'bf16':
        return affine_act(conv(x, w, nbr, inv, n_out, need_dx=need_dx), scale, shift, act=act, res=res)
    h16 = torch.bfloat16
    y16 = bool(out_bf16 and cout % 4 == 0)
    x16, r16 = x.d.dtype == h16, (res is not None and res.d.dtype == h16)
    y = Var(empty((n_out, cout), x.d, dtype=h16 if y16 else torch.float32))
    ic = (img is not None and K == 9 and x16 and res is None and act in (0, 1) and cin == cout and _ld(x.d) == cin
          and hip.raw('es_img_conv3_supported')(img[0], img[1], img[2], cin, img[3], 0) == 1)
    if ic and hip.try_call('es_img_conv3_bf16', P(x.d), cin, P(w.bf16()[1]), img[0], img[1], img[2], cin, img[3], 0, P(scale), P(shift), 0,
                           0, act, P(y.d), int(y16), cout, _stream()):
        entry = 'es_img_conv3_bf16'
    elif x16 or r16 or y16:
        call('es_spconv_fwd_bf16_io', P(x.d), int(x16), _ld(x.d), P(w.bf16()[1]), P(nbr), n_out, n_in, K, cin, cout, P(scale),
             P(shift), P(res.d) if res is not None else 0, int(r16), _ld(res.d) if res is not None else 0, act, P(y.d),
             int(y16), cout, _stream())
        entry = 'es_spconv_fwd_bf16_io'
    else:
        call('es_spconv_fwd_bf16_affine', P(x.d), _ld(x.d), P(w.bf16()[1]), P(nbr), n_out, n_in, K, cin, cout, P(scale),
             P(shift), P(res.d) if res is not None else 0, _ld(res.d) if res is not None else 0, act, P(y.d), cout, _stream())
        entry = 'es_spconv_fwd_bf16_affine'
    if y16:
        y.dh = y.d
    if x16:
        x.dh = x.d
    if DEBUG_FWD is not None:
        fwd_record('conv_affine', entry, x=x.d, w=w, nbr=nbr, n_out=n_out, round=True, scale=scale, shift=shift,
                   res=res.d if res is not None else None, act=act, y=y.d)

    if act == 1 and res is None:
        y.gate = scale
    gate = x.gate if sole_consumer else None

    def bwd():
        if y.g is None:
            return
        if DEBUG_GRADS is not None:
            DEBUG_GRADS[id(y)] = y.g.clone()
        if y.gated:
            gconv = y.g
        else:
            gr = accr = 0
            if res is not None and res.rg:
                t, accr = _grad_target(res, res.d)
                gr = P(t)
            gconv = torch.empty((n_out, cout), dtype=torch.float32, device=y.d.device)
            call('es_affine_act_bwd_yh' if y.d.dtype == h16 else 'es_affine_act_bwd', P(y.g), P(y.d), P(scale), n_out, cout, act,
                 P(gconv), 0, gr, accr, _stream())
        _conv_backward(x, w, nbr, inv, n_out, y, gconv, None, 0, need_dx, True, gate, img=img)
    TAPE.add(bwd)
    return y


def gen_conv_transpose(x, w):
    K, cin, cout = w.d.shape
    n = x.d.shape[0]
    y = Var(empty((n * 8, cout), x.d))
    s = _stream()
    bf = PRECISION[0] == 'bf16'
    fused = False
    if bf and GEN_FUSED[0] and x.d.dtype == torch.float32:
        fused = hip.raw('es_gen_transpose_fwd_bf16')(P(x.d), _ld(x.d), P(w.bf16()[1]), n, cin, cout, P(y.d), s) == 0
    for k in range(0 if not fused else 8, 8):
        if bf:
            call('es_spconv_fwd_bf16', P(x.d), 0, _ld(x.d), w.bf16()[1].data_ptr() + 2 * k * cin * cout, 0, n, n, 1, cin,
                 cout, 0, y.d.data_ptr() + 4 * k * cout, 8 * cout, 0, s)
        else:
            call('es_spconv_fwd', P(x.d), _ld(x.d), w.d.data_ptr() + 4 * k * cin * cout, 0, n, n, 1, cin, cout, 0,
                 y.d.data_ptr() + 4 * k * cout, 8 * cout, 0, 0, s)
    if DEBUG_FWD is not None:
        fwd_record('gen_transpose', 'es_gen_transpose_fwd_bf16' if fused else ('es_spconv_fwd_bf16' if bf else 'es_spconv_fwd'),
                   x=x.d, w=w, round=bf, y=y.d)

# ... 494 lines not shown
```

### embodiedscan_amd/hip.py

```python
import ctypes
import os
import re

_HERE = os.path.dirname(os.path.abspath(__file__))
LIB_PATH = os.path.join(_HERE, 'libes_hip.so')
HEADER_PATH = os.path.join(os.path.dirname(_HERE), 'include', 'es_hip.h')

_CT = {'int': ctypes.c_int, 'float': ctypes.c_float, 'double': ctypes.c_double, 'size_t': ctypes.c_size_t}


def parse_header(path=HEADER_PATH):
    src = open(path).read()
    src = re.sub(r'/\*.*?\*/', ' ', src, flags=re.S)
    out = {}
    for m in re.finditer(r'\b(int|size_t)\s+(es_\w+)\s*\(([^)]*)\)\s*;', src):
        ret, name, args = m.group(1), m.group(2), m.group(3)
        at, an = [], []
        for a in args.split(','):
            a = a.strip()
            if not a or a == 'void':
                continue
            an.append(re.findall(r'(\w+)\s*$', a)[0])
            if '*' in a:
                at.append(ctypes.c_void_p)
            else:
                toks = [t for t in a.split() if t != 'const']
                at.append(_CT[toks[0]])
        out[name] = (_CT[ret], at, an)
    return out


PROTOS = parse_header()
CONSTS = {k: int(v) for k, v in re.findall(r'#define\s+(ES_\w+)\s+(\d+)', open(HEADER_PATH).read())}

if not os.path.exists(LIB_PATH):
    raise ImportError(f'{LIB_PATH} is missing: build it with `make -C embodiedscan_amd/csrc` '
                      '(or __graft_entry__.build()); there is no CPU fallback for the HIP path')
_lib = ctypes.CDLL(LIB_PATH)
_fn = {}
for _name, (_ret, _at, _an) in PROTOS.items():
    _f = getattr(_lib, _name)
    _f.restype, _f.argtypes = _ret, _at
    _fn[_name] = _f


if os.environ.get('ES_PINGPONG') is not None:
    _fn['es_set_option'](1, int(os.environ['ES_PINGPONG']))
if os.environ.get('ES_WGRAD_HUGE') is not None:
    _fn['es_set_option'](2, int(os.environ['ES_WGRAD_HUGE']))
if os.environ.get('ES_ROWGEMM') is not None:
    _fn['es_set_option'](3, int(os.environ['ES_ROWGEMM']))
for _key, _env in ((4, 'ES_WG_BIG_TARGET'), (5, 'ES_WG_BIG_ROWS'), (6, 'ES_WG_SMALL_TARGET'), (7, 'ES_WG_CAP_MB'), (8, 'ES_FWD_SPLIT_WGS'),
                  (10, 'ES_DMA'), (11, 'ES_DMA_MIN_CIN'), (12, 'ES_RG128_MIN_CIN'), (14, 'ES_WGRAD_TR'), (15, 'ES_NORM_CB_ROWS'),
                  (16, 'ES_SPLIT_FOLD'), (19, 'ES_RG128_MIN_WGS'), (20, 'ES_WSHARE'), (21, 'ES_NARROW'), (23, 'ES_RG320'), (24, 'ES_LIN_SMALL'), (25, 'ES_EXPAND'), (26, 'ES_EXPAND_WGS')):
    if os.environ.get(_env) is not None:
        _fn['es_set_option'](_key, int(os.environ[_env]))


class HipError(RuntimeError):
    pass


PROFILE = None
PAIRS = {}


def register_map(nbr):
    if PROFILE is not None and nbr is not None:
        PAIRS[nbr.data_ptr()] = (nbr >= 0).sum()
    return nbr


_EXT_STREAMS = {}


def _stream_of(handle):
    import torch
    st = _EXT_STREAMS.get(handle)
    if st is None:
        st = _EXT_STREAMS[handle] = torch.cuda.ExternalStream(handle) if handle else torch.cuda.default_stream()
    return st


def _launch(name, args):
    prof = PROFILE
    if prof is not None and name in prof['names']:
        e0, e1 = prof['event'](), prof['event']()
        st = _stream_of(args[-1])
        e0.record(st)
        rc = _fn[name](*args)
        e1.record(st)
        if rc == 0:
            prof['records'].append((name, e0, e1, args))
    else:
        rc = _fn[name](*args)
    return rc


def call(name, *args):
    rc = _launch(name, args)
    if rc != 0:
        raise HipError(f'{name} failed with status {rc}')


def try_call(name, *args):
    rc = _launch(name, args)
    if rc not in (0, -4):
        raise HipError(f'{name} failed with status {rc}')
    return rc == 0


def raw(name):
    return _fn[name]


_STREAM = [None]
_STREAM_OBJ = [None]


def stream():
    if _STREAM[0] is None:
        refresh_stream()
    return _STREAM[0]


def refresh_stream():
    import torch
    _STREAM_OBJ[0] = torch.cuda.current_stream()
    _STREAM[0] = _STREAM_OBJ[0].cuda_stream
    return _STREAM[0]


def stream_obj():
    if _STREAM_OBJ[0] is None:
        refresh_stream()
    return _STREAM_OBJ[0]


def P(t):
# ... 14 lines not shown
```

### embodiedscan_amd/models/backbones/mink_resnet.py

```python
from ... import engine as E
from ...registry import MODELS
from ...sparse import SparseTensor
from ..dense_heads.fcaf3d_head import _BN


@MODELS.register_module()
class MinkResNet:
    arch_settings = {18: (2, 2, 2, 2), 34: (3, 4, 6, 3)}

    def __init__(self, depth, in_channels, num_stages=4, pool=True):
        if depth not in self.arch_settings:
            raise KeyError(f'invalid depth {depth} for the BasicBlock MinkResNet implemented here')
        assert 4 >= num_stages >= 1
        self.depth, self.in_channels, self.num_stages, self.pool = depth, in_channels, num_stages, pool
        self.stage_blocks = self.arch_settings[depth][:num_stages]
        self.training = True
        self.trace = None

    def bind(self, arena, prefix='backbone_3d.'):
        self.arena, self.prefix = arena, prefix
        par = lambda n: E.Param(arena.p[prefix + n], arena.g.get(prefix + n))
        self.conv1 = par('conv1.kernel')
        self.norm1 = (par('norm1.weight'), par('norm1.bias'))
        self.blocks = []
        for li, nblk in enumerate(self.stage_blocks):
            layer = []
            for bi in range(nblk):
                p = f'layer{li + 1}.{bi}.'
                blk = dict(conv1=par(p + 'conv1.kernel'), norm1=_BN(arena, prefix + p + 'norm1'),
                           conv2=par(p + 'conv2.kernel'), norm2=_BN(arena, prefix + p + 'norm2'))
                if bi == 0:
                    blk['down'] = (par(p + 'downsample.0.kernel'), _BN(arena, prefix + p + 'downsample.1'))
                layer.append(blk)
            self.blocks.append(layer)
        return self

    def prefetch_coords(self, cs):
        from ... import sparse as _sp
        sets = _sp.strided_chain(cs, 1 + int(bool(self.pool)) + len(self.blocks))
        sets[0].offsets()
        outs = sets[1 + int(bool(self.pool)):]
        for o in outs:
            o.offsets()
        return outs

    def prefetch_maps(self, cs):
        o1 = cs.strided(2)
        cs.kernel_map(o1, 3)
        if self.pool:
            o2 = o1.strided(2)
            o1.kernel_map(o2, 2)
            cs = o2
        else:
            cs = o1
        for layer in self.blocks:
            oc = cs.strided(2)
            for k in (3, 1):
                cs.kernel_map(oc, k)
                cs.inverse_map(oc, k)
            cs = oc
            cs.kernel_map(cs, 3)
            cs.inverse_map(cs, 3)

    def forward(self, x):
        tr = self.training
        cs = x.cs
        o1 = cs.strided(2)
        f = E.conv(x.F, self.conv1, cs.kernel_map(o1, 3), cs.inverse_map(o1, 3), o1.n, need_dx=x.F.rg)
        f = E.norm(f, self.norm1[0], self.norm1[1], o1.offsets(), 1e-8, act=1)
        if self.pool:
            o2 = o1.strided(2)
            f = E.maxpool(f, o1.kernel_map(o2, 2), o2.n)
            cs = o2
        else:
            cs = o1
        outs = []
        for layer in self.blocks:
            for bi, blk in enumerate(layer):
                if bi == 0:
                    oc = cs.strided(2)
                    o = E.conv(f, blk['conv1'], cs.kernel_map(oc, 3), cs.inverse_map(oc, 3), oc.n)
                    idt = E.conv(f, blk['down'][0], cs.kernel_map(oc, 1), cs.inverse_map(oc, 1), oc.n)
                    idt = blk['down'][1](idt, act=0, training=tr)
                    cs = oc
                else:
                    o = E.conv(f, blk['conv1'], cs.kernel_map(cs, 3), cs.inverse_map(cs, 3), cs.n)
                    idt = f
                c1 = o
                o = blk['norm1'](o, act=1, training=tr)
                n1 = o
                o = E.conv(o, blk['conv2'], cs.kernel_map(cs, 3), cs.inverse_map(cs, 3), cs.n)
                f = blk['norm2'](o, act=1, res=idt, training=tr)
                if self.trace is not None:
                    self.trace += [c1, n1, o, f]
            outs.append(SparseTensor(cs, f))
        return outs

    __call__ = forward
```

### embodiedscan_amd/models/dense_heads/fcaf3d_head.py

```python
import torch
from ... import hip
from ... import engine as E
from ... import sparse
from ...geometry import euler_to_matrix_zxy
from ...hip import P, call, iarr, farr, parr
from ...parallel import reduce_mean
from ...registry import MODELS
from ...sparse import SparseTensor


def _stream():
    return hip.stream()


def upload_gts(gts, dev):
    Gs = [int(b.shape[0]) for b, _ in gts]
    tot = sum(Gs)
    host = torch.empty(max(tot, 1) * 19, dtype=torch.float32, pin_memory=dev.type == 'cuda')
    hb, hr, hl = host[:tot * 9].view(tot, 9), host[tot * 9:tot * 18].view(tot, 9), host[tot * 18:tot * 19].view(torch.int32)
    a = 0
    for (b, l), G in zip(gts, Gs):
        if G:
            bh = b.detach().float().cpu()
            hb[a:a + G] = bh
            hr[a:a + G] = euler_to_matrix_zxy(-bh[:, 6:9]).reshape(G, 9)
            hl[a:a + G] = l.detach().to(torch.int32).cpu()
        a += G
    d = host.to(dev, non_blocking=True)
    db, dr, dl = d[:tot * 9].view(tot, 9), d[tot * 9:tot * 18].view(tot, 9), d[tot * 18:tot * 19].view(torch.int32)
    out, a = [], 0
    for G in Gs:
        out.append((db[a:a + G], dr[a:a + G], dl[a:a + G]))
        a += G
    return out


def get_targets_device(points_per_level, gt_boxes, gt_labels, assign_thr, center_thr, dev_gt=None):
    if isinstance(points_per_level, tuple):
        points, level_off = points_per_level
    else:
        points = torch.cat(points_per_level)
        level_off = [0]
        for p in points_per_level:
            level_off.append(level_off[-1] + int(p.shape[0]))
    dev = points.device
    N, G = int(points.shape[0]), int(gt_boxes.shape[0])
    if dev_gt is not None:
        boxes, rot, labels = dev_gt
    else:
        boxes_h = gt_boxes.detach().float().cpu()
        rot_neg = euler_to_matrix_zxy(-boxes_h[:, 6:9]).reshape(G, 9) if G else torch.zeros((0, 9))
        boxes = boxes_h.to(dev).contiguous()
        rot = rot_neg.to(dev).contiguous()
        labels = gt_labels.detach().to(torch.int32).to(dev).contiguous()
    n_lvl = len(level_off) - 1
    scratch = torch.empty(max(G, 1) * max(N, 1) + (n_lvl + 2) * max(G, 1) + 8, dtype=torch.float32, device=dev)
    center_t = torch.empty(N, dtype=torch.float32, device=dev)
    bbox_t = torch.empty((N, 9), dtype=torch.float32, device=dev)
    cls_t = torch.empty(N, dtype=torch.int32, device=dev)
    box_idx = torch.empty(N, dtype=torch.int32, device=dev)
    n_pos = torch.empty(1, dtype=torch.int32, device=dev)
    call('es_get_targets', P(points), N, iarr(level_off), n_lvl, P(boxes), P(rot), P(labels), G, int(assign_thr),
         int(center_thr), P(scratch), P(center_t), P(bbox_t), P(cls_t), P(box_idx), P(n_pos), _stream())
    return center_t, bbox_t, cls_t, box_idx, n_pos


class _BN:
    def __init__(self, arena, prefix):
        g = arena.g
        self.w = E.Param(arena.p[prefix + '.bn.weight'], g.get(prefix + '.bn.weight'))
        self.b = E.Param(arena.p[prefix + '.bn.bias'], g.get(prefix + '.bn.bias'))
        self.running = (arena.p[prefix + '.bn.running_mean'], arena.p[prefix + '.bn.running_var'])

    def __call__(self, x, act=0, res=None, training=True):
        n = x.d.shape[0]
        if training:
            return E.norm(x, self.w, self.b, [0, n], 1e-5, act=act, res=res, running=self.running)
        C = self.w.d.numel()
        sc, sh = torch.empty(C, dtype=torch.float32, device=x.d.device), torch.empty(C, dtype=torch.float32, device=x.d.device)
        call('es_bn_fold', P(self.w.d), P(self.b.d), P(self.running[0]), P(self.running[1]), C, 1e-5, P(sc), P(sh), _stream())
        y = E.Var(torch.empty_like(x.d), rg=False)
        call('es_affine_act_fwd', P(x.d), P(sc), P(sh), P(res.d) if res is not None else 0, n, C, act, P(y.d), _stream())
        return y


def conv3(st, w, out_set=None):
    cs = st.cs
    nbr, inv = cs.kernel_map(cs, 3), cs.inverse_map(cs, 3)
    return SparseTensor(cs, E.conv(st.F, w, nbr, inv, cs.n))


@MODELS.register_module()
class FCAF3DHeadRotMat:
    def __init__(self, num_classes, in_channels, out_channels, num_reg_outs, voxel_size, pts_prune_threshold,
                 pts_assign_threshold, pts_center_threshold, center_loss=None, bbox_loss=None, cls_loss=None,
                 decouple_bbox_loss=False, decouple_groups=3, decouple_weights=None, norm_decouple_loss=False,
                 train_cfg=None, test_cfg=None, init_cfg=None):
        self.num_classes, self.in_channels, self.out_channels = num_classes, tuple(in_channels), out_channels
        self.num_reg_outs = num_reg_outs
        self.voxel_size = voxel_size
        self.pts_prune_threshold = pts_prune_threshold
        self.pts_assign_threshold = pts_assign_threshold
        self.pts_center_threshold = pts_center_threshold
        center_loss = center_loss or dict(type='mmdet.CrossEntropyLoss', use_sigmoid=True)
        bbox_loss = bbox_loss or dict(type='BBoxCDLoss', mode='l1', loss_weight=1.0, group='g8')
        cls_loss = cls_loss or dict(type='mmdet.FocalLoss')
        assert center_loss.get('type') == 'mmdet.CrossEntropyLoss' and center_loss.get('use_sigmoid', False)
        assert bbox_loss.get('type') == 'BBoxCDLoss' and bbox_loss.get('mode', 'l2') == 'l1' and \
            bbox_loss.get('group', 'g8') == 'g8'
        assert cls_loss.get('type') == 'mmdet.FocalLoss'
        assert num_reg_outs == 12, 'only the 6D-rotation (12 output) coder is implemented'
        self.bbox_loss_weight = float(bbox_loss.get('loss_weight', 1.0))
        self.focal_gamma, self.focal_alpha = float(cls_loss.get('gamma', 2.0)), float(cls_loss.get('alpha', 0.25))
        self.decouple_bbox_loss = decouple_bbox_loss
        self.decouple_groups = decouple_groups
        assert not norm_decouple_loss, 'norm_decouple_loss is not used by the shipped configs'
        if decouple_weights is None:
            decouple_weights = [1.0 / decouple_groups] * decouple_groups
        self.decouple_weights = list(decouple_weights)
        self.train_cfg, self.test_cfg = train_cfg, test_cfg
        self.training = True

    def bind(self, arena, prefix='bbox_head.'):
        g = arena.g
        self.arena, self.prefix = arena, prefix
        par = lambda n: E.Param(arena.p[prefix + n], g.get(prefix + n))
        n_lvl = len(self.in_channels)
        self.up, self.out = {}, {}
        for i in range(n_lvl):
            if i > 0:
                p = f'up_block_{i}'
                self.up[i] = (par(p + '.0.kernel'), _BN(arena, prefix + p + '.1'), par(p + '.3.kernel'),
                              _BN(arena, prefix + p + '.4'))
            p = f'out_block_{i}'
            self.out[i] = (par(p + '.0.kernel'), _BN(arena, prefix + p + '.1'))
        self.head_w = par('head_out.kernel')
        self.head_b = par('head_out.bias')
        self.scales = [par(f'scales.{i}.scale') for i in range(n_lvl)]
        return self

    def _prune(self, x, score_set, score):
        off = x.cs.offsets()
        thr = self.pts_prune_threshold
        if all(off[b + 1] - off[b] <= thr for b in range(x.cs.n_batch)):
            return x
        idx, w = sparse.interp_map(x.cs, score_set)
        s = torch.empty(x.cs.n, dtype=torch.float32, device=x.cs.device)
        call('es_interp_scores', P(score), P(idx), P(w), x.cs.n, P(s), _stream())
        mask = torch.empty(x.cs.n, dtype=torch.int32, device=x.cs.device)
        ws, nws = E.ticket_ws(int(hip.raw('es_topk_mask_workspace_ints')(x.cs.n_batch)), s, tag='topk')
        call('es_topk_mask_ws', P(s), iarr(off), x.cs.n_batch, int(thr), P(mask), P(ws), nws, _stream())
        kept = [0]
        for b in range(x.cs.n_batch):
            kept.append(kept[-1] + min(off[b + 1] - off[b], thr))
        new_set, src = sparse.compact(x.cs, mask, offsets=kept)
        return SparseTensor(new_set, E.gather_rows(x.F, src))

    def prefetch_coords(self, level_sets, maps=False):
        x = level_sets[-1]
        thr = self.pts_prune_threshold
        if maps:
            x.kernel_map(x, 3), x.inverse_map(x, 3)
        for i in range(len(level_sets) - 2, -1, -1):
            c = x.children()
            if maps:
                c.kernel_map(c, 3), c.inverse_map(c, 3)
            u, _, _ = sparse.union(c, level_sets[i])
            off = u.offsets()
            if any(off[b + 1] - off[b] > thr for b in range(u.n_batch)):
                break
            if maps:
                u.kernel_map(u, 3), u.inverse_map(u, 3)
            x = u

    def _levels(self, inputs):
        n_lvl = len(inputs)
        levels = [None] * n_lvl
        x = inputs[-1]
        score_set = score = None
        tr = self.training
        for i in range(n_lvl - 1, -1, -1):
            if i < n_lvl - 1:
                wt, bn1, wc, bn2 = self.up[i + 1]
                y = SparseTensor(x.cs.children(), bn1(E.gen_conv_transpose(x.F, wt), act=2, training=tr))
                y = conv3(y, wc)
                y = SparseTensor(y.cs, bn2(y.F, act=2, training=tr))
                u, pa, pb = sparse.union(y.cs, inputs[i].cs)
                x = SparseTensor(u, E.union_add(y.F, inputs[i].F, pa, pb, u.n))
                x = self._prune(x, score_set, score)
            wo, bno = self.out[i]
            out = conv3(x, wo)
            out = SparseTensor(out.cs, bno(out.F, act=2, training=tr))
            n = out.cs.n
            ho = E.conv(out.F, self.head_w, None, None, n, bias=self.head_b, bias_from=13)
            ncol = ho.d.shape[1]
            bbox = torch.empty((n, 12), dtype=torch.float32, device=ho.d.device)
            call('es_reg_decode_fwd', ho.d.data_ptr() + 4, ncol, n, P(self.scales[i].d), P(bbox), _stream())
            if i > 0:
                score = torch.empty(n, dtype=torch.float32, device=ho.d.device)
                call('es_row_max', ho.d.data_ptr() + 4 * 13, ncol, n, self.num_classes, P(score), _stream())
                score_set = out.cs
            levels[i] = dict(cs=out.cs, ho=ho, bbox=bbox, scale=self.scales[i], out=out.F, x=x.F)
        return levels

    def forward(self, x):
        levels = self._levels(x)
        cp, bp, kp, pts = [], [], [], []
        for lv in levels:
            off = lv['cs'].offsets()
            ho, bbox = lv['ho'].d, lv['bbox']
            points = torch.empty((lv['cs'].n, 3), dtype=torch.float32, device=ho.device)
            call('es_coords_to_points', P(lv['cs'].coords), lv['cs'].n, float(self.voxel_size), P(points), _stream())
            sl = [slice(off[b], off[b + 1]) for b in range(lv['cs'].n_batch)]
            cp.append([ho[s, 0:1] for s in sl])
            bp.append([bbox[s] for s in sl])
            kp.append([ho[s, 13:13 + self.num_classes] for s in sl])
            pts.append([points[s] for s in sl])
        return cp, bp, kp, pts

    __call__ = forward

    def predict(self, x, batch_data_samples, rescale=False):
        from ...structures import EulerDepthInstance3DBoxes, InstanceData
        cfg = self.test_cfg or {}
        nms_pre, score_thr, iou_thr = cfg.get('nms_pre', 1000), cfg.get('score_thr', 0.01), cfg.get('iou_thr', 0.5)
        prev = E.TAPE.enabled
        E.TAPE.enabled = False
        try:
            levels = self._levels(x)
        finally:
            E.TAPE.enabled = prev
        dev = levels[0]['ho'].d.device
        s = _stream()
        B = levels[0]['cs'].n_batch
        C = self.num_classes
        per_level = []
        for lv in levels:
            n = lv['cs'].n
            ho = lv['ho'].d
            scores = torch.empty((n, C), dtype=torch.float32, device=dev)
            maxs = torch.empty(n, dtype=torch.float32, device=dev)
            call('es_predict_scores', P(ho), ho.shape[1], n, C, P(scores), P(maxs), s)
            pts = torch.empty((n, 3), dtype=torch.float32, device=dev)
            call('es_coords_to_points', P(lv['cs'].coords), n, float(self.voxel_size), P(pts), s)
            off = lv['cs'].offsets()
            mask = torch.empty(n, dtype=torch.int32, device=dev)
            call('es_topk_mask', P(maxs), iarr(off), B, int(nms_pre) if nms_pre > 0 else n + 1, P(mask), s)
            kept_set, src = sparse.compact(lv['cs'], mask)
            boxes = torch.empty((kept_set.n, 9), dtype=torch.float32, device=dev)
            call('es_decode_boxes', P(pts), P(lv['bbox']), P(src), kept_set.n, P(boxes), s)
            sc_k = torch.empty((kept_set.n, C), dtype=torch.float32, device=dev)
            call('es_row_move', P(sc_k), C, P(scores), C, P(src), kept_set.n, C, 0, s)
            per_level.append((kept_set.offsets(), boxes, sc_k))
        results = []
        for b in range(B):
# ... 129 lines not shown
```

### embodiedscan_amd/models/necks/mink_neck.py

```python
import torch
from ... import engine as E
from ... import hip
from ... import sparse
from ...hip import P, call, iarr
from ...registry import MODELS
from ...sparse import SparseTensor
from ..dense_heads.fcaf3d_head import _BN, conv3


@MODELS.register_module()
class MinkNeck:
    def __init__(self, num_classes, in_channels, out_channels, voxel_size, pts_prune_threshold, train_cfg=None,
                 test_cfg=None, init_cfg=None):
        self.num_classes, self.in_channels, self.out_channels = num_classes, tuple(in_channels), out_channels
        self.voxel_size, self.pts_prune_threshold = voxel_size, pts_prune_threshold
        self.training = True

    def bind(self, arena, prefix='neck_3d.'):
        par = lambda n: E.Param(arena.p[prefix + n], arena.g.get(prefix + n))
        self.up, self.out = {}, {}
        for i in range(len(self.in_channels)):
            if i > 0:
                p = f'up_block_{i}'
                self.up[i] = (par(p + '.0.kernel'), _BN(arena, prefix + p + '.1'), par(p + '.3.kernel'), _BN(arena, prefix + p + '.4'))
            p = f'out_block_{i}'
            self.out[i] = (par(p + '.0.kernel'), _BN(arena, prefix + p + '.1'))
        self.cls_w, self.cls_b = arena.p[prefix + 'conv_cls.kernel'], arena.p[prefix + 'conv_cls.bias']
        return self

    def _prune(self, x, score_set, score):
        off = x.cs.offsets()
        thr = self.pts_prune_threshold
        if all(off[b + 1] - off[b] <= thr for b in range(x.cs.n_batch)):
            return x
        idx, w = sparse.interp_map(x.cs, score_set)
        s = torch.empty(x.cs.n, dtype=torch.float32, device=x.cs.device)
        call('es_interp_scores', P(score), P(idx), P(w), x.cs.n, P(s), hip.stream())
        mask = torch.empty(x.cs.n, dtype=torch.int32, device=x.cs.device)
        ws, nws = E.ticket_ws(int(hip.raw('es_topk_mask_workspace_ints')(x.cs.n_batch)), s, tag='topk')
        call('es_topk_mask_ws', P(s), iarr(off), x.cs.n_batch, int(thr), P(mask), P(ws), nws, hip.stream())
        kept = [0]
        for b in range(x.cs.n_batch):
            kept.append(kept[-1] + min(off[b + 1] - off[b], thr))
        new_set, src = sparse.compact(x.cs, mask, offsets=kept)
        return SparseTensor(new_set, E.gather_rows(x.F, src))

    def prefetch_coords(self, level_sets, maps=False):
        x = level_sets[-1]
        thr = self.pts_prune_threshold
        if maps:
            x.kernel_map(x, 3), x.inverse_map(x, 3)
        for i in range(len(level_sets) - 2, -1, -1):
            c = x.children()
            if maps:
                c.kernel_map(c, 3), c.inverse_map(c, 3)
            u, _, _ = sparse.union(c, level_sets[i])
            off = u.offsets()
            if any(off[b + 1] - off[b] > thr for b in range(u.n_batch)):
                break
            if maps:
                u.kernel_map(u, 3), u.inverse_map(u, 3)
            x = u

    def levels(self, inputs):
        n_lvl = len(inputs)
        res = [None] * n_lvl
        x = inputs[-1]
        score_set = score = None
        tr = self.training
        for i in range(n_lvl - 1, -1, -1):
            if i < n_lvl - 1:
                wt, bn1, wc, bn2 = self.up[i + 1]
                y = SparseTensor(x.cs.children(), bn1(E.gen_conv_transpose(x.F, wt), act=2, training=tr))
                y = conv3(y, wc)
                y = SparseTensor(y.cs, bn2(y.F, act=2, training=tr))
                u, pa, pb = sparse.union(y.cs, inputs[i].cs)
                x = SparseTensor(u, E.union_add(y.F, inputs[i].F, pa, pb, u.n))
                x = self._prune(x, score_set, score)
            wo, bno = self.out[i]
            out = conv3(x, wo)
            out = SparseTensor(out.cs, bno(out.F, act=2, training=tr))
            n = out.cs.n
            cls = torch.empty((n, self.num_classes), dtype=torch.float32, device=out.F.d.device)
            call('es_spconv_fwd', P(out.F.d), out.F.d.stride(0), P(self.cls_w), 0, n, n, 1, self.out_channels, self.num_classes,
                 P(self.cls_b), P(cls), self.num_classes, 0, 0, hip.stream())
            if E.DEBUG_FWD is not None:
                E.fwd_record('conv', 'es_spconv_fwd', x=out.F.d, xh=None, w=self.cls_w.view(1, self.out_channels, self.num_classes), nbr=None,
                             n_out=n, bias=self.cls_b, round=False, y=cls)
            score = torch.empty(n, dtype=torch.float32, device=cls.device)
            call('es_row_max', P(cls), self.num_classes, n, self.num_classes, P(score), hip.stream())
            score_set = out.cs
            res[i] = dict(cs=out.cs, out=out.F, cls=cls)
        return res

    def forward(self, x, batch_size):
        lv = self.levels(x)
        B = batch_size
        order = list(range(len(lv) - 1, -1, -1))
        offs = {i: lv[i]['cs'].offsets() for i in order}
        lens = [sum(offs[i][b + 1] - offs[i][b] for i in order) for b in range(B)]
        Lmax = max(lens)
        C = self.out_channels
        dev = lv[0]['out'].d.device
        feats = torch.zeros((B * Lmax, C), dtype=torch.float32, device=dev)
        pts = torch.zeros((B * Lmax, 3), dtype=torch.float32, device=dev)
        scores = torch.zeros((B * Lmax, self.num_classes), dtype=torch.float32, device=dev)
        maps = []
        pos = [0] * B
        s = hip.stream()
        for i in order:
            n = lv[i]['cs'].n
            dst = torch.empty(n, dtype=torch.int32)
            for b in range(B):
                r0, r1 = offs[i][b], offs[i][b + 1]
                dst[r0:r1] = torch.arange(b * Lmax + pos[b], b * Lmax + pos[b] + (r1 - r0), dtype=torch.int32)
                pos[b] += r1 - r0
            dst = dst.to(dev, non_blocking=True)
            p = torch.empty((n, 3), dtype=torch.float32, device=dev)
            call('es_coords_to_points', P(lv[i]['cs'].coords), n, float(self.voxel_size), P(p), s)
            call('es_row_move', P(feats), C, P(lv[i]['out'].d), C, P(dst), n, C, 2, s)
            call('es_row_move', P(pts), 3, P(p), 3, P(dst), n, 3, 2, s)
            call('es_row_move', P(scores), self.num_classes, P(lv[i]['cls']), self.num_classes, P(dst), n, self.num_classes, 2, s)
            maps.append((lv[i]['out'], dst, n))
        fv = E.Var(feats)

        def bwd():
            if fv.g is None:
                return
            for out, dst, n in maps:
                g = torch.empty_like(out.d)
                call('es_row_move', P(g), C, P(fv.g), C, P(dst), n, C, 0, hip.stream())
                if out.g is None:
                    out.g = g
                else:
                    E.add_into(out.g, g)
        E.TAPE.add(bwd)
        self.last = dict(feats=fv, points=pts, scores=scores, lens=lens, Lmax=Lmax, levels=lv)
        fl = [feats[b * Lmax:b * Lmax + lens[b]] for b in range(B)]
        sl = [scores[b * Lmax:b * Lmax + lens[b]] for b in range(B)]
        pl = [pts[b * Lmax:b * Lmax + lens[b]] for b in range(B)]
        return fl, sl, pl

    __call__ = forward
```

### embodiedscan_amd/sparse.py

```python
import ctypes
import weakref

import torch
from . import hip
from .hip import P, call


def _stream():
    return hip.stream()


_PIN = {}


def _pinned_ints(n=64):
    t = _PIN.get('buf')
    if t is None or t.numel() < n:
        t = torch.empty(max(n, 256), dtype=torch.int32)
        if torch.cuda.is_available():
            t = t.pin_memory()
        _PIN['buf'] = t
    return t


def read_ints(dev_tensor):
    n = dev_tensor.numel()
    pin = _pinned_ints(n)
    pin[:n].copy_(dev_tensor.reshape(-1), non_blocking=True)
    torch.cuda.current_stream(dev_tensor.device).synchronize()
    return [int(v) for v in pin[:n].tolist()]


def _pow2_cap(n):
    c = 1024
    while c < 2 * n + 2:
        c *= 2
    return c


class CoordSet:

    def __init__(self, keys, n, ts, n_batch, tkeys=None, tvals=None):
        self.keys, self.n, self.ts, self.n_batch = keys, int(n), int(ts), int(n_batch)
        self.tkeys, self.tvals = tkeys, tvals
        self._coords = None
        self._off_dev = None
        self._off_host = None
        self.cache = {}

    @property
    def device(self):
        return self.keys.device

    def table(self):
        if self.tkeys is None:
            cap = _pow2_cap(self.n)
            self.tkeys = torch.empty(cap, dtype=torch.int64, device=self.device)
            self.tvals = torch.empty(cap, dtype=torch.int32, device=self.device)
            call('es_build_table', P(self.keys), self.n, P(self.tkeys), P(self.tvals), cap, _stream())
        return self.tkeys, self.tvals, self.tkeys.numel()

    @property
    def coords(self):
        if self._coords is None:
            self._coords = torch.empty((self.n, 4), dtype=torch.int32, device=self.device)
            call('es_keys_to_coords', P(self.keys), self.n, P(self._coords), _stream())
        return self._coords

    def offsets_dev(self):
        if self._off_dev is None:
            self._off_dev = torch.empty(self.n_batch + 1, dtype=torch.int32, device=self.device)
            call('es_batch_offsets', P(self.keys), self.n, self.n_batch, P(self._off_dev), _stream())
        return self._off_dev

    def offsets(self):
        if self._off_host is None:
            self._off_host = read_ints(self.offsets_dev())
        return self._off_host

    def strided(self, stride):
        key = ('stride', stride)
        if key not in self.cache:
            out_ts = self.ts * stride
            tmp = torch.empty(self.n, dtype=torch.int64, device=self.device)
            call('es_stride_keys', P(self.keys), self.n, out_ts, P(tmp), _stream())
            self.cache[key] = unique_first(tmp, self.n, out_ts, self.n_batch)[0]
        return self.cache[key]

    def _cached(self, key, partner):
        e = self.cache.get(key)
        return e[0] if (e is not None and e[1]() is partner) else None

    def kernel_map(self, out, ksize):
        key = ('kmap', id(out), ksize)
        nbr = self._cached(key, out)
        if nbr is None:
            tk, tv, cap = self.table()
            K = ksize ** 3
            nbr = torch.empty((out.n, K), dtype=torch.int32, device=self.device)
            call('es_kernel_map', P(out.keys), out.n, P(tk), P(tv), cap, ksize, self.ts, P(nbr), _stream())
            self.cache[key] = (hip.register_map(nbr), weakref.ref(out))
        return nbr

    def inverse_map(self, out, ksize):
        key = ('imap', id(out), ksize)
        inv = self._cached(key, out)
        if inv is None:
            nbr = self.kernel_map(out, ksize)
            K = ksize ** 3
            inv = torch.empty((self.n, K), dtype=torch.int32, device=self.device)
            call('es_inverse_map', P(nbr), out.n, K, self.n, P(inv), _stream())
            if out is self and ksize % 2 == 1:
                inv._mirror_of = nbr
            self.cache[key] = (hip.register_map(inv), weakref.ref(out))
        return inv

    def children(self):
        if 'gen' not in self.cache:
            keys = torch.empty(self.n * 8, dtype=torch.int64, device=self.device)
            call('es_gen_children_keys', P(self.keys), self.n, self.ts // 2, P(keys), _stream())
            self.cache['gen'] = CoordSet(keys, self.n * 8, self.ts // 2, self.n_batch)
        return self.cache['gen']


COORD_BATCH = [__import__('os').environ.get('ES_COORD_BATCH', '1') != '0']


def strided_chain(root, n_levels):
    have, cur = [], root
    for _ in range(n_levels):
        nxt = cur.cache.get(('stride', 2))
        if nxt is None:
            break
        have.append(nxt)
        cur = nxt
    if len(have) == n_levels:
        return have
    dev, n, B = root.device, root.n, root.n_batch
    if not COORD_BATCH[0] or n <= 0 or have:
        out, cur = [], root
        for _ in range(n_levels):
            cur = cur.strided(2)
            out.append(cur)
        return out
    cap = _pow2_cap(n)
    ts = [root.ts * (2 ** (l + 1)) for l in range(n_levels)]
    tk = [torch.empty(cap, dtype=torch.int64, device=dev) for _ in range(n_levels)]
    tv = [torch.empty(cap, dtype=torch.int32, device=dev) for _ in range(n_levels)]
    ok = [torch.empty(n, dtype=torch.int64, device=dev) for _ in range(n_levels)]
    tmp = torch.empty(n, dtype=torch.int64, device=dev)
    scratch = torch.empty(2 * n + n // 2048 + 8, dtype=torch.int32, device=dev)
    per = B + 2
    res = torch.empty(n_levels * per, dtype=torch.int32, device=dev)
    res_host = _pinned_ints(n_levels * per)
    ptrs = lambda ts_: (ctypes.c_void_p * n_levels)(*[t.data_ptr() for t in ts_])
    call('es_strided_chain', P(root.keys), n, B, n_levels, (ctypes.c_int * n_levels)(*ts), P(tmp), P(scratch), ptrs(tk), ptrs(tv),
         (ctypes.c_int * n_levels)(*([cap] * n_levels)), ptrs(ok), P(res), res_host.data_ptr(), _stream())
    res_host = res_host[:n_levels * per].tolist()
    out, cur = [], root
    for l in range(n_levels):
        m = int(res_host[l * per])
        cs = CoordSet(ok[l][:m], m, ts[l], B, tk[l], tv[l])
        cs._off_dev = res[l * per + 1:(l + 1) * per]
        cs._off_host = [int(res_host[l * per + 1 + b]) for b in range(B + 1)]
        cur.cache[('stride', 2)] = cs
        out.append(cs)
        cur = cs
    return out


def unique_first(keys, n, ts, n_batch, want_src=True):
    dev = keys.device
    cap = _pow2_cap(n)
    tkeys = torch.empty(cap, dtype=torch.int64, device=dev)
    tvals = torch.empty(cap, dtype=torch.int32, device=dev)
    scratch = torch.empty(2 * n + n // 2048 + 8, dtype=torch.int32, device=dev)
    out_keys = torch.empty(max(n, 1), dtype=torch.int64, device=dev)
    out_src = torch.empty(max(n, 1), dtype=torch.int32, device=dev)
    cnt = _pinned_ints()
    call('es_unique_first', P(keys), n, P(tkeys), P(tvals), cap, P(scratch), P(out_keys), P(out_src),
         cnt.data_ptr(), _stream())
    m = int(cnt[0])
    return CoordSet(out_keys[:m], m, ts, n_batch, tkeys, tvals), out_src[:m]


def voxelize(points, voxel_size):
    dev = points[0].device
    n = sum(int(p.shape[0]) for p in points)
    keys = torch.empty(n, dtype=torch.int64, device=dev)
    o = 0
    for b, p in enumerate(points):
        assert p.dtype == torch.float32 and p.stride(1) == 1
        call('es_voxel_keys', P(p), p.shape[0], p.stride(0), b, float(voxel_size), keys.data_ptr() + 8 * o, _stream())
        o += int(p.shape[0])
    cs, src = unique_first(keys, n, 1, len(points))
    return morton_sorted(cs, src)


def voxelize_range(points, range_min, voxel_size, clamp_max):
    dev = points[0].device
    n = sum(int(p.shape[0]) for p in points)
    keys = torch.empty(n, dtype=torch.int64, device=dev)
    rng = hip.farr(list(range_min) + list(voxel_size) + [float(c) for c in clamp_max])
    o = 0
    for b, p in enumerate(points):
# ... 95 lines not shown
```

### include/es_hip.h

```cpp
#ifndef ES_HIP_H
#define ES_HIP_H
#include <stddef.h>
#include <stdint.h>
#ifdef __cplusplus
extern "C" {
#endif

#define ES_MAX_SEG 32

#define ES_MAX_BATCH 512
int es_voxel_keys(const float* points, int n, int ld, int batch, float voxel_size, int64_t* keys, void* stream);
int es_unique_first(const int64_t* keys, int n, int64_t* tkeys, int* tvals, int cap, int* scratch,
                    int64_t* out_keys, int* out_src, int* count_host, void* stream);
size_t es_sort_scratch_bytes(int n);
int es_morton_sort(const int64_t* keys, const int* src, int n, void* scratch, size_t scratch_bytes, int64_t* out_keys,
                   int* out_src, void* stream);
int es_sort_u64(const int64_t* keys, const int* src, int n, void* scratch, size_t scratch_bytes, int64_t* out_keys, int* out_src,
                void* stream);
int es_draw_keys(const float* depth, int V, int HW, size_t seed, float* values, int64_t* keys, void* stream);
int es_draw_keys_index(int n, size_t seed, int stream_id, float* values, int64_t* keys, void* stream);
int es_draw_unpack(const int64_t* keys, int n, const int* in_view, const int* in_pix, int* out_view, int* out_pix, void* stream);
int es_build_table(const int64_t* keys, int n, int64_t* tkeys, int* tvals, int cap, void* stream);
int es_stride_keys(const int64_t* in_keys, int n, int out_ts, int64_t* out_keys, void* stream);
int es_keys_to_coords(const int64_t* keys, int n, int* coords , void* stream);
// ... 52 lines not shown

size_t es_norm_workspace_floats(int n, int C, const int* seg_off_host, int nseg);
int es_norm_fwd(const float* x, int ldx, int n, int C, const int* seg_off_host, int nseg, float eps,
                const float* weight, const float* bias, const float* res, int ldr, int act, float* running_mean,
                float* running_var, float momentum, float* mean, float* invstd, float* workspace, float* y, int ldy,
                void* y_bf16, void* stream);
int es_norm_bwd(float* dy, int ldd, const float* y, int ldy, const float* x, int ldx, int n, int C,
                const int* seg_off_host, int nseg, const float* mean, const float* invstd, const float* weight,
                int act, float* dweight, float* dbias, float* workspace, float* dx, int ldo, int accumulate,
                void* dx_bf16, void* stream);
int es_maxpool_fwd(const float* x, int ldx, const int* nbr, int n_out, int K, int C, float* y, int* arg, void* stream);
int es_maxpool_fwd_h(const float* x, int ldx, const int* nbr, int n_out, int K, int C, void* y_bf16, void* stream);
int es_maxpool_bwd(const float* dy, const int* arg, int n_out, int C, float* dx, int ldo, void* stream);
int es_row_move(float* dst, int ldd, const float* src, int lds, const int* idx, int n, int C, int mode, void* stream);
int es_axpy2d(float* dst, int ldd, const float* src, int lds, int n, int C, float alpha, int op, void* stream);
int es_interp_scores(const float* score, const int* idx, const float* w, int n, float* out, void* stream);
size_t es_colsum_workspace_floats(int n, int C);
int es_colsum(const float* g, int ld, int n, int C, float* dst, int accumulate, float* workspace, size_t workspace_floats, void* stream);
int es_topk_mask(const float* values, const int* seg_off_host, int nseg, int k, int* mask, void* stream);
size_t es_topk_mask_workspace_ints(int nseg);
int es_topk_mask_ws(const float* values, const int* seg_off_host, int nseg, int k, int* mask, int* workspace, size_t workspace_ints,
                    void* stream);
int es_row_max(const float* x, int ldx, int n, int C, float* out, void* stream);
int es_bn_fold(const float* w, const float* b, const float* rm, const float* rv, int C, float eps, float* scale,
               float* shift, void* stream);
int es_affine_act_fwd(const float* x, const float* scale, const float* shift, const float* res, size_t n, int C,
                      int act, float* y, void* stream);
int es_affine_act_bwd(const float* dy, const float* y, const float* scale, size_t n, int C, int act, float* dx,
                      int acc_x, float* dres, int acc_r, void* stream);
int es_affine_act_bwd_yh(const float* dy, const void* y_bf16, const float* scale, size_t n, int C, int act, float* dx,
                         int acc_x, float* dres, int acc_r, void* stream);

#define ES_FUSE_NOPS 0
#define ES_FUSE_OPS 1
#define ES_FUSE_ROTINV 9
#define ES_FUSE_ISCALE 18
#define ES_FUSE_NTRANS 19
#define ES_FUSE_SFX 22
#define ES_FUSE_SFY 23
#define ES_FUSE_CROPX 24
#define ES_FUSE_CROPY 25
#define ES_FUSE_FLIP 26
#define ES_FUSE_ORIW 27
#define ES_FUSE_PADW 28
#define ES_FUSE_PADH 29
#define ES_FUSE_PROJ 32
int es_point_sample_fwd(const int* coords, int n, float voxel_size, const float* meta, int meta_stride, int V,
                        const float* feats , int Hf, int Wf, int C, float* out, int ldo,
                        int* pix , int* cnt , void* stream);
int es_point_sample_fwd_h(const int* coords, int n, float voxel_size, const float* meta, int meta_stride, int V,
                          const void* feats_bf16, int Hf, int Wf, int C, float* out, int ldo, int* pix, int* cnt, void* stream);
int es_point_sample_fwd_pts(const int* coords, const float* points, int n, const float* meta, int meta_stride, int V,
                            const float* feats, int Hf, int Wf, int C, float* out, int ldo, int* pix, int* cnt,
                            void* stream);
int es_point_sample_bwd(const int* coords, int n, int V, const float* dout, int ldo, const int* pix, const int* cnt,
                        int Hf, int Wf, int C, float* dfeats, int n_img, int* head, int* next, int accumulate, void* stream);
int es_point_sample_win_fwd(const int* coords, int n, float voxel_size, const float* meta, int meta_stride, int V, const int* win,
                            const float* feats, int Hf, int Wf, int C, float* out, int ldo, int* pix, int* cnt, void* stream);
int es_point_sample_win_fwd_h(const int* coords, int n, float voxel_size, const float* meta, int meta_stride, int V, const int* win,
                              const void* feats_bf16, int Hf, int Wf, int C, float* out, int ldo, int* pix, int* cnt, void* stream);
int es_point_sample_win_bwd(const int* coords, int n, int V, const int* win, const float* dout, int ldo, const int* pix,
                            const int* cnt, int Hf, int Wf, int C, float* dfeats, int n_img, int* head, int* next, int accumulate,
                            void* stream);
int es_point_sample_prefix_fwd_pts(const int* coords, const float* points, int n, const float* meta, int meta_stride, int V,
                                   const float* feats, int Hf, int Wf, int C, float* out, int ldo, int* pix, int* cnt,
                                   void* stream);
int es_point_sample_step_fwd_pts(const int* coords, const float* points, int n, const float* meta, int meta_stride,
                                 const float* feats, int Hf, int Wf, int C, float* sum, int* nvalid, float* out, int ldo,
                                 int* pix, void* stream);
int es_point_sample_prefix_bwd(const int* coords, int n, int V, const float* dout, int ldo, const int* pix, const int* cnt,
                               int Hf, int Wf, int C, float* dfeats, int n_img, int* head, int* next, int accumulate,
                               void* stream);

int es_get_targets(const float* points, int N, const int* level_off_host, int n_levels, const float* boxes,
                   const float* rot_neg, const int* labels, int G, int assign_thr, int center_thr, float* scratch,
                   float* center_t, float* bbox_t, int* cls_t, int* box_idx, int* n_pos_dev, void* stream);

int es_focal_loss(const float* logits, int ldl, const int* labels, int N, int C, float gamma, float alpha,
                  const float* avg_factor_dev, float grad_scale, float* grad, int ldg, double* partial ,
                  float* loss_out , void* stream);
int es_focal_loss_clear(const float* logits, int ldl, const int* labels, int N, int C, float gamma, float alpha,
                        const float* avg_factor_dev, float grad_scale, float* grad, int ldg, double* partial ,
                        float* loss_out , int lead, int tail, void* stream);
int es_reg_decode_fwd(const float* reg, int ldr, int n, const float* scale, float* bbox , void* stream);
int es_reg_decode_bwd(const float* reg, int ldr, const float* bbox, const float* dbbox, int n, const float* scale,
                      float* dreg, int ldg, float* dscale, float* partial, void* stream);
#define ES_MAX_LEVELS 8
int es_pos_losses(const int* cls_t, int n, const int* n_pos_dev, int max_pos, int* pos_ws, const float* points,
                  int n_levels, const int* level_off_host, const void* const* ho_host, const void* const* bbox_host,
                  void* const* dho_host, void* const* dbbox_host, int ldh, const float* center_t, const float* bbox_t,
                  const float* avg_factor_dev, float grad_scale, const float* group_w_host, double* loss_acc ,
                  void* stream);

int es_predict_scores(const float* ho, int ldh, int n, int C, float* scores , float* max_scores, void* stream);
int es_decode_boxes(const float* points, const float* bbox, const int* idx, int m, float* out, void* stream);
int es_nms3d_multiclass(const float* boxes, const float* scores, int M, int C, float score_thr, float iou_thr,
                        int* keep_idx, int* keep_cnt, void* stream);

int es_grad_norm(const float* grad, size_t n, double* partial , float* norm_out, void* stream);
int es_adamw_step(float* param, const float* grad, float* exp_avg, float* exp_avg_sq, size_t n, float lr, float beta1,
                  float beta2, float eps, float weight_decay, int step, float max_norm, const float* grad_norm_dev,
                  float grad_scale, void* stream);
int es_adamw_table(float* param, const float* grad, float* exp_avg, float* exp_avg_sq, const void* table_dev, int n_entries,
                   int total_items, double lr, float beta1, float beta2, float eps, double weight_decay, int step, float max_norm,
                   const float* grad_norm_dev, float grad_scale, void* stream);
int es_sumsq_partial(const float* grad, size_t n, double* partial , void* stream);
int es_norm_from_partials(const double* partial, int n_partials, float scale, float* norm_out, void* stream);

int es_depth_to_points(const float* depth, int H, int W, const int* sel_view, const int* sel_pix, int n,
                       const float* mats , const float* aug , float* out, void* stream);
int es_stem_conv_fwd(const float* x, const float* w, const float* scale, const float* shift, int n_img, int H, int W,
                     int Cout, float* y, void* stream);
int es_stem_pool_fwd(const float* x, const float* w, const float* scale, const float* shift, int n_img, int H, int W,
                     int Cout, void* y_bf16, void* stream);
int es_preprocess_img(const unsigned char* img, int n_img, int H, int W, int Hp, int Wp, int flip,
                      const float* mean_host, const float* std_host, float pad_value,
                      float* out , void* stream);

int es_resize_u8(const unsigned char* src, int V, int H, int W, const int* xofs, const short* ialpha, const int* yofs,
                 const short* ibeta, int h, int w, unsigned char* dst, void* stream);

int es_volume_map(int n_batch, int X, int Y, int Z, int Xo, int Yo, int Zo, int ksize, int stride, int pad, int* nbr,
                  void* stream);
int es_volume_up_index(int n_batch, int X, int Y, int Z, int* idx, void* stream);
int es_voxel_keys_range(const float* points, int n, int ld, int batch, const float* rng_host, int64_t* keys, void* stream);
int es_dense_index(const int* coords, int n, int ts, int X, int Y, int Z, int* idx, void* stream);
int es_upsample_nearest_add_fwd(float* fine, const float* coarse, int n_img, int Hf, int Wf, int Hc, int Wc, int C,
                                void* stream);
int es_upsample_nearest_add_bwd(const float* dfine, float* dcoarse, int n_img, int Hf, int Wf, int Hc, int Wc, int C,
                                int accumulate, void* stream);
int es_row_argmax(const float* x, int ldx, int n, int C, int* out, void* stream);
int es_occ_targets(const int* gt_occ, int n, int ratio, int X, int Y, int Z, const unsigned char* mask,
                   int* winner_scratch, int* gt, void* stream);
int es_occ_loss(const float* logits, int ld, const int* gt, int n, int C, float weight, double* stats, float* coeff,
                float* dlogits, int ldg, float* loss_out, float* total_acc, void* stream);

int es_attn_fwd(const float* Q, int ldq, const float* K, int ldk, const float* V, int ldv, int B, int H, int Lq, int Lk,
                const int* klen_dev, float* O, int ldo, float* lse, int bf16, void* stream);
size_t es_attn_kv_bytes(int H, int Lk, int bf16);
int es_attn_kv_prepare(const float* K, int ldk, const float* V, int ldv, int H, int Lk, int bf16, void* kv, void* stream);
int es_attn_kv_fwd(const float* Q, int ldq, const void* kv, int H, int Lq, int Lk, float* O, int ldo, float* lse, int bf16,
                   void* stream);
size_t es_rows_scatter_sum_workspace_ints(int P, int L);
int es_rows_scatter_sum(const float* dy, int ldy, const int* idx, int P, int Q, int L, int C, float* dx, int ldx, int accumulate,
                        int* workspace, size_t workspace_ints, void* stream);
int es_attn_bwd(const float* Q, int ldq, const float* K, int ldk, const float* V, int ldv, const float* O, int ldo,
                const float* dO, int ldd, const float* lse, int B, int H, int Lq, int Lk, const int* klen_dev,
                float* delta_scratch, float* dQ, int ldgq, float* dK, int ldgk, float* dV, int ldgv, int accumulate, int bf16,
                void* stream);
size_t es_attn_kv_bwd_workspace_bytes(int H, int Lq, int bf16);
int es_attn_kv_bwd(const float* Q, int ldq, const float* K, int ldk, const float* V, int ldv, const float* O, int ldo,
                   const float* dO, int ldd, const float* lse, int H, int Lq, int Lk, float* delta_scratch, void* workspace,
                   size_t workspace_bytes, float* dQ, int ldgq, float* dK, int ldgk, float* dV, int ldgv, int accumulate, int bf16,
                   void* stream);
int es_layernorm_fwd(const float* x, const float* res, int n, int C, const float* w, const float* b, float eps, float* y,
                     float* z, float* mean, float* rstd, void* stream);
size_t es_layernorm_bwd_workspace_floats(int n, int C);
int es_layernorm_bwd(const float* dy, const float* z, int n, int C, const float* w, const float* mean, const float* rstd,
                     float* dz, int accumulate, float* dw, float* db, float* workspace, size_t workspace_floats, void* stream);
int es_text_embed_ln(const long long* ids, int B, int T, int pad_id, const float* word, const float* pos, const float* type0,
                     int C, int vocab, int max_pos, const float* ln_w, const float* ln_b, float eps, float* y, int* pos_ids,
                     void* stream);
int es_text_add_ln(const float* x, const float* res, int n, int C, const float* w, const float* b, float eps, float* y,
                   void* stream);
int es_bias_gelu(float* x, int ld, int n, int C, const float* bias, void* stream);
int es_text_attn_fwd(const float* qkv, int ld, int B, int H, int T, const int* mask_dev, float* O, int ldo, int bf16,
// ... 86 lines not shown
```

Measured before the change: 180.8 scans/s.

## Mirror self-inverse kernel maps, add bitmap halo planner and prefetching focal loss

For stride-1 odd-kernel convolutions onto the same coordinate set, the inverse map is replaced by the forward map read with the tap index mirrored (k -> K-1-k), so building and storing a separate inverse map is skipped. The mirror flag is threaded through the spconv, narrow and bf16 io kernels. Separately, the halo planner gets a bitmap-plus-prefix-count path that replaces the LDS hash table and O(n^2) ranking when the index span fits, falling back to hashing otherwise. The focal loss gets a variant that holds up to 5 logits per lane and prefetches the next row. This adds complexity and depends on the neighbour map truly being symmetric.

New measurement: 183.4 scans/s (median of 6 runs). +1.5%, better.

```diff
diff --git a/embodiedscan_amd/csrc/halo.hip b/embodiedscan_amd/csrc/halo.hip
--- a/embodiedscan_amd/csrc/halo.hip
+++ b/embodiedscan_amd/csrc/halo.hip
@@ -21,19 +21,10 @@
 
 __device__ __attribute__((aligned(16))) unsigned short g_hl_zero[8];
 
-__global__ __launch_bounds__(512) void k_halo_plan(const int* __restrict__ nbr, int n_out, int K,
-                                                   unsigned short* __restrict__ loc, int* __restrict__ hrows,
-                                                   int* __restrict__ hcnt) {
+__device__ __forceinline__ void halo_plan_stage(const int* __restrict__ nbr, int n_out, int K, int tile, int* nb) {
   constexpr int NE = HL_BM * HL_K;
-  __shared__ __attribute__((aligned(16))) int nb[NE];
-  __shared__ unsigned short slotOf[NE];
-  __shared__ int hk[HL_HT];
-  __shared__ unsigned short hv[HL_HT];
-  __shared__ int cnt;
-  const int t = threadIdx.x, tile = blockIdx.x;
+  const int t = threadIdx.x;
   const long long e0 = (long long)tile * NE, eN = (long long)n_out * K;
-  for (int i = t; i < HL_HT; i += 512) hk[i] = -1;
-  if (t == 0) cnt = 0;
   for (int i = t; i < NE / 4; i += 512) {
     int4 v = make_int4(-1, -1, -1, -1);
     const long long e = e0 + (long long)i * 4;
@@ -45,7 +36,11 @@
     }
     ((int4*)nb)[i] = v;
   }
-  __syncthreads();
+}
+__device__ __forceinline__ void halo_plan_hash(int tile, int* nb, unsigned short* slotOf, int* hk, unsigned short* hv, int* cntp,
+                                               unsigned short* __restrict__ loc, int* __restrict__ hrows, int* __restrict__ hcnt) {
+  constexpr int NE = HL_BM * HL_K;
+  const int t = threadIdx.x;
   for (int e = t; e < NE; e += 512) {
     const int v = nb[e];
     unsigned short so = 0xFFFFu;
@@ -66,7 +61,7 @@
     const int v = hk[sl];
     const unsigned long long m = __ballot(v >= 0);
     int base = 0;
-    if ((t & 63) == 0 && m) base = atomicAdd(&cnt, __popcll(m));
+    if ((t & 63) == 0 && m) base = atomicAdd(cntp, __popcll(m));
     base = __shfl(base, 0, 64);
     if (v >= 0) {
       const int pos = base + __popcll(m & ((1ull << (t & 63)) - 1ull));
@@ -75,7 +70,7 @@
     }
   }
   __syncthreads();
-  const int nU = cnt;
+  const int nU = *cntp;
   unsigned short* const rk = (unsigned short*)hk;
   int* const hr = hrows + (size_t)tile * NE;
   for (int i = t; i < nU; i += 512) {
@@ -94,14 +89,133 @@
     dst[i] = p0 | (p1 << 16);
   }
 }
+__global__ __launch_bounds__(512) void k_halo_plan(const int* __restrict__ nbr, int n_out, int K,
+                                                   unsigned short* __restrict__ loc, int* __restrict__ hrows,
+                                                   int* __restrict__ hcnt) {
+  constexpr int NE = HL_BM * HL_K;
+  __shared__ __attribute__((aligned(16))) int nb[NE];
+  __shared__ unsigned short slotOf[NE];
+  __shared__ int hk[HL_HT];
+  __shared__ unsigned short hv[HL_HT];
+  __shared__ int cnt;
+  const int t = threadIdx.x, tile = blockIdx.x;
+  for (int i = t; i < HL_HT; i += 512) hk[i] = -1;
+  if (t == 0) cnt = 0;
+  halo_plan_stage(nbr, n_out, K, tile, nb);
+  __syncthreads();
+  halo_plan_hash(tile, nb, slotOf, hk, hv, &cnt, loc, hrows, hcnt);
+}
+
+#define HL_SPAN (1 << 19)
+#define HL_WORDS (HL_SPAN / 32)
+__global__ __launch_bounds__(512) void k_halo_plan_bitmap(const int* __restrict__ nbr, int n_out, int K,
+                                                          unsigned short* __restrict__ loc, int* __restrict__ hrows,
+                                                          int* __restrict__ hcnt) {
+  constexpr int NE = HL_BM * HL_K;
+  constexpr int OFF_BM = NE * 4, OFF_PRE = OFF_BM + HL_WORDS * 4, OFF_END = OFF_PRE + HL_WORDS * 2;
+  static_assert(OFF_BM + NE * 2 + HL_HT * 4 + HL_HT * 2 <= OFF_END, "the hash path's tables live in the bitmap's LDS");
+  __shared__ __attribute__((aligned(16))) unsigned char smem[OFF_END];
+  __shared__ int redMin[8], redMax[8], wtot[8];
+  __shared__ int cnt;
+  int* const nb = (int*)smem;
+  unsigned int* const bm = (unsigned int*)(smem + OFF_BM);
+  unsigned short* const pre = (unsigned short*)(smem + OFF_PRE);
+  const int t = threadIdx.x, lane = t & 63, wv = t >> 6, tile = blockIdx.x;
+  halo_plan_stage(nbr, n_out, K, tile, nb);
+  __syncthreads();
+  int mn = 0x7FFFFFFF, mx = -1;
+  for (int e = t; e < NE; e += 512) {
+    const int v = nb[e];
+    if (v >= 0) { mn = min(mn, v); mx = max(mx, v); }
+  }
+#pragma unroll
+  for (int d = 32; d >= 1; d >>= 1) {
+    mn = min(mn, __shfl_xor(mn, d, 64));
+    mx = max(mx, __shfl_xor(mx, d, 64));
+  }
+  if (lane == 0) { redMin[wv] = mn; redMax[wv] = mx; }
+  __syncthreads();
+#pragma unroll
+  for (int w = 0; w < 8; ++w) { mn = min(mn, redMin[w]); mx = max(mx, redMax[w]); }
+  const long long span = mx >= 0 ? (long long)mx - mn + 1 : 0;
+  if (span > HL_SPAN) {
+    unsigned short* const slotOf = (unsigned short*)(smem + OFF_BM);
+    int* const hk = (int*)(smem + OFF_BM + NE * 2);
+    unsigned short* const hv = (unsigned short*)(smem + OFF_BM + NE * 2 + HL_HT * 4);
+    for (int i = t; i < HL_HT; i += 512) hk[i] = -1;
+    if (t == 0) cnt = 0;
+    __syncthreads();
+    halo_plan_hash(tile, nb, slotOf, hk, hv, &cnt, loc, hrows, hcnt);
+    return;
+  }
+  const int nW = (int)((span + 31) >> 5);
+  for (int w = t; w < nW; w += 512) bm[w] = 0u;
+  __syncthreads();
+  for (int e = t; e < NE; e += 512) {
+    const int v = nb[e];
+    if (v >= 0) atomicOr(&bm[(unsigned)(v - mn) >> 5], 1u << ((v - mn) & 31));
+  }
+  __syncthreads();
+  const int per = (nW + 511) >> 9;
+  const int w0 = t * per, w1 = min(nW, w0 + per);
+  int mine = 0;
+  for (int w = w0; w < w1; ++w) mine += __popc(bm[w]);
+  int inc = mine;
+#pragma unroll
+  for (int d = 1; d < 64; d <<= 1) {
+    const int o = __shfl_up(inc, d, 64);
+    if (lane >= d) inc += o;
+  }
+  if (lane == 63) wtot[wv] = inc;
+  __syncthreads();
+  int run = inc - mine;
+  int nU = 0;
+#pragma unroll
+  for (int w = 0; w < 8; ++w) {
+    if (w < wv) run += wtot[w];
+    nU += wtot[w];
+  }
+  int* const hr = hrows + (size_t)tile * NE;
+  for (int w = w0; w < w1; ++w) {
+    unsigned int bits = bm[w];
+    pre[w] = (unsigned short)run;
+    while (bits) {
+      const int b = __ffsll((unsigned long long)bits) - 1;
+      bits &= bits - 1u;
+      hr[run++] = mn + w * 32 + b;
+    }
+  }
+  if (t == 0) hcnt[tile] = nU;
+  __syncthreads();
+  unsigned int* const dst = (unsigned int*)(loc + (size_t)tile * NE);
+  for (int i = t; i < NE / 2; i += 512) {
+    unsigned int p[2];
+#pragma unroll
+    for (int h = 0; h < 2; ++h) {
+      const int v = nb[2 * i + h];
+      p[h] = 0xFFFFu;
+      if (v >= 0) {
+        const unsigned int o = (unsigned int)(v - mn);
+        p[h] = (unsigned int)pre[o >> 5] + (unsigned int)__popc(bm[o >> 5] & ((1u << (o & 31)) - 1u));
+      }
+    }
+    dst[i] = p[0] | (p[1] << 16);
+  }
+}
+
+static int ES_OPT_HALO_PLAN_BITMAP = 1;
 
 extern "C" size_t es_halo_plan_rows(int n_out) { return (size_t)es_cdiv(n_out, HL_BM) * HL_BM; }
 
 extern "C" int es_halo_plan(const int* nbr, int n_out, int K, void* loc, int* hrows, int* hcnt, void* stream) {
   if (n_out <= 0) return 0;
   if (K != HL_K || nbr == nullptr) return -4;
-  hipLaunchKernelGGL(k_halo_plan, dim3(es_cdiv(n_out, HL_BM)), dim3(512), 0, (hipStream_t)stream, nbr, n_out, K,
-                     (unsigned short*)loc, hrows, hcnt);
+  if (ES_OPT_HALO_PLAN_BITMAP)
+    hipLaunchKernelGGL(k_halo_plan_bitmap, dim3(es_cdiv(n_out, HL_BM)), dim3(512), 0, (hipStream_t)stream, nbr, n_out, K,
+                       (unsigned short*)loc, hrows, hcnt);
+  else
+    hipLaunchKernelGGL(k_halo_plan, dim3(es_cdiv(n_out, HL_BM)), dim3(512), 0, (hipStream_t)stream, nbr, n_out, K,
+                       (unsigned short*)loc, hrows, hcnt);
   ES_CHECK_LAUNCH();
   return 0;
 }
@@ -322,6 +436,7 @@
 extern "C" int es_halo_set_option(int key, int value) {
   if (key == 30) { ES_OPT_HALO_MIN_WGS = value; return 0; }
   if (key == 31) { ES_OPT_HALO_WGS = value; return 0; }
+  if (key == 32) { ES_OPT_HALO_PLAN_BITMAP = value; return 0; }
   return -1;
 }
 
diff --git a/embodiedscan_amd/csrc/losses.hip b/embodiedscan_amd/csrc/losses.hip
--- a/embodiedscan_amd/csrc/losses.hip
+++ b/embodiedscan_amd/csrc/losses.hip
@@ -1,6 +1,21 @@
 #include "common.h"
 #include "../../include/es_hip.h"
 
+__device__ __forceinline__ void focal_elem(float x, bool pos, bool g2, float gamma, float alpha, float& l, float& g) {
+  float p = 1.f / (1.f + expf(-x));
+  if (pos) {
+    float q = 1.f - p;
+    float lp = logf(fmaxf(p, 1.17549435e-38f));
+    float w = g2 ? q * q : powf(q, gamma);
+    l = -alpha * w * lp;
+    g = -alpha * w * (1.f - p - gamma * p * lp);
+  } else {
+    float ln = logf(fmaxf(1.f - p, 1.17549435e-38f));
+    float w = g2 ? p * p : powf(p, gamma);
+    l = -(1.f - alpha) * w * ln;
+    g = -(1.f - alpha) * w * (gamma * (1.f - p) * ln - p);
+  }
+}
 __global__ __launch_bounds__(256) void k_focal(const float* __restrict__ logits, int ldl,
                                                const int* __restrict__ labels, int N, int C, float gamma,
                                                float alpha, const float* __restrict__ avg_factor, float grad_scale,
@@ -16,23 +31,73 @@
     float* grow = grad ? grad + (size_t)i * ldg : nullptr;
     float acc = 0.f;
     for (int c = lane; c < C; c += 64) {
-      float x = row[c];
-      float p = 1.f / (1.f + expf(-x));
       float l, g;
-      if (lab == c) {
-        float q = 1.f - p;
-        float lp = logf(fmaxf(p, 1.17549435e-38f));
-        float w = g2 ? q * q : powf(q, gamma);
-        l = -alpha * w * lp;
-        g = -alpha * w * (1.f - p - gamma * p * lp);
-      } else {
-        float ln = logf(fmaxf(1.f - p, 1.17549435e-38f));
-        float w = g2 ? p * p : powf(p, gamma);
-        l = -(1.f - alpha) * w * ln;
-        g = -(1.f - alpha) * w * (gamma * (1.f - p) * ln - p);
-      }
+      focal_elem(row[c], lab == c, g2, gamma, alpha, l, g);
       acc += l;
       if (grow) grow[c] = g * inv;
+    }
+    if (grow) {
+      for (int c = lane; c < lead; c += 64) grow[c - lead] = 0.f;
+      for (int c = lane; c < tail; c += 64) grow[C + c] = 0.f;
+    }
+    s += (double)acc;
+  }
+  s = es_wave_sum_d(s);
+  if (lane == 0) red[threadIdx.x >> 6] = s;
+  __syncthreads();
+  if (threadIdx.x == 0) partial[blockIdx.x] = red[0] + red[1] + red[2] + red[3];
+}
+#define FOCAL_SLOTS 5
+__global__ __launch_bounds__(256) void k_focal_inflight(const float* __restrict__ logits, int ldl,
+                                                        const int* __restrict__ labels, int N, int C, float gamma,
+                                                        float alpha, const float* __restrict__ avg_factor, float grad_scale,
+                                                        float* __restrict__ grad, int ldg, double* __restrict__ partial, int lead,
+                                                        int tail) {
+  __shared__ double red[4];
+  const float inv = grad_scale / (avg_factor[0] + 1.1920929e-07f);
+  const bool g2 = gamma == 2.f;
+  const int lane = threadIdx.x & 63;
+  const int step = gridDim.x * 4;
+  double s = 0.0;
+  int i = blockIdx.x * 4 + (threadIdx.x >> 6);
+  float xn[FOCAL_SLOTS];
+  int labn = 0;
+#pragma unroll
+  for (int j = 0; j < FOCAL_SLOTS; ++j) xn[j] = 0.f;
+  if (i < N) {
+    const float* row = logits + (size_t)i * ldl;
+    labn = labels[i];
+#pragma unroll
+    for (int j = 0; j < FOCAL_SLOTS; ++j) {
+      const int c = lane + 64 * j;
+      if (c < C) xn[j] = row[c];
+    }
+  }
+  for (; i < N; i += step) {
+    float x[FOCAL_SLOTS];
+    const int lab = labn;
+#pragma unroll
+    for (int j = 0; j < FOCAL_SLOTS; ++j) x[j] = xn[j];
+    if (i + step < N) {
+      const float* row = logits + (size_t)(i + step) * ldl;
+      labn = labels[i + step];
+#pragma unroll
+      for (int j = 0; j < FOCAL_SLOTS; ++j) {
+        const int c = lane + 64 * j;
+        if (c < C) xn[j] = row[c];
+      }
+    }
+    float* grow = grad ? grad + (size_t)i * ldg : nullptr;
+    float acc = 0.f;
+#pragma unroll
+    for (int j = 0; j < FOCAL_SLOTS; ++j) {
+      const int c = lane + 64 * j;
+      if (c < C) {
+        float l, g;
+        focal_elem(x[j], lab == c, g2, gamma, alpha, l, g);
+        acc += l;
+        if (grow) grow[c] = g * inv;
+      }
     }
     if (grow) {
       for (int c = lane; c < lead; c += 64) grow[c - lead] = 0.f;
@@ -59,6 +124,11 @@
   }
 }
 #define FOCAL_BLOCKS 2048
+static int ES_OPT_FOCAL_INFLIGHT = 1;
+extern "C" int es_losses_set_option(int key, int value) {
+  if (key == 40) { ES_OPT_FOCAL_INFLIGHT = value; return 0; }
+  return -2;
+}
 extern "C" int es_focal_loss(const float* logits, int ldl, const int* labels, int N, int C, float gamma, float alpha,
                              const float* avg_factor_dev, float grad_scale, float* grad, int ldg, double* partial,
                              float* loss_out, void* stream) {
@@ -73,8 +143,12 @@
   int g = es_cdiv(N, 4);
   if (g > FOCAL_BLOCKS) g = FOCAL_BLOCKS;
   if (g < 1) g = 1;
-  hipLaunchKernelGGL(k_focal, dim3(g), dim3(256), 0, st, logits, ldl, labels, N, C, gamma, alpha, avg_factor_dev,
-                     grad_scale, grad, ldg, partial, lead, tail);
+  if (ES_OPT_FOCAL_INFLIGHT && C <= 64 * FOCAL_SLOTS)
+    hipLaunchKernelGGL(k_focal_inflight, dim3(g), dim3(256), 0, st, logits, ldl, labels, N, C, gamma, alpha, avg_factor_dev,
+                       grad_scale, grad, ldg, partial, lead, tail);
+  else
+    hipLaunchKernelGGL(k_focal, dim3(g), dim3(256), 0, st, logits, ldl, labels, N, C, gamma, alpha, avg_factor_dev,
+                       grad_scale, grad, ldg, partial, lead, tail);
   hipLaunchKernelGGL(k_sum_partials, dim3(1), dim3(256), 0, st, partial, g, avg_factor_dev, loss_out);
   ES_CHECK_LAUNCH();
   return 0;
diff --git a/embodiedscan_amd/csrc/spconv.hip b/embodiedscan_amd/csrc/spconv.hip
--- a/embodiedscan_amd/csrc/spconv.hip
+++ b/embodiedscan_amd/csrc/spconv.hip
@@ -80,6 +80,8 @@
 
   const int t = threadIdx.x, lane = t & 63, wv = t >> 6;
   const int row0 = blockIdx.x * BM, n0 = blockIdx.y * BN;
+  const int mirror = accumulate & 2;
+  accumulate &= 1;
   const bool vecA = ((ldx & 3) == 0) && ((((uintptr_t)X) & 15) == 0);
   const bool vecB = TRANS_W ? (((Cin & 3) == 0) && ((((uintptr_t)W) & 15) == 0))
                             : (((Cout & 3) == 0) && ((((uintptr_t)W) & 15) == 0));
@@ -89,7 +91,7 @@
   for (int e = t; e < BM * K; e += 256) {
     int r = e / K, k = e - r * K;
     int j = row0 + r, v = -1;
-    if (j < n_out) v = nbr ? nbr[(size_t)j * K + k] : (j < n_in ? j : -1);
+    if (j < n_out) v = nbr ? nbr[(size_t)j * K + (mirror ? K - 1 - k : k)] : (j < n_in ? j : -1);
     nbrS[e] = v;
     if (v >= 0) tapAny[k] = 1;
   }
@@ -233,7 +235,7 @@
 #endif
 template <int CIN>
 __device__ __forceinline__ void narrow_stage(const float* __restrict__ X, int ldx, const int* __restrict__ nbr, int row0,
-                                             int n_out, int n_in, float* xg, int* idxS, int* maskS) {
+                                             int n_out, int n_in, float* xg, int* idxS, int* maskS, int mirror = 0) {
   const int t = threadIdx.x;
   constexpr int NI = (NW_ROWS * 27 + 255) / 256;
   int v[NI];
@@ -241,7 +243,7 @@
   for (int i = 0; i < NI; ++i) {
     const int e = t + i * 256;
     v[i] = -1;
-    if (e < NW_ROWS * 27 && row0 + e / 27 < n_out) v[i] = nbr[(size_t)row0 * 27 + e];
+    if (e < NW_ROWS * 27 && row0 + e / 27 < n_out) v[i] = nbr[(size_t)row0 * 27 + (mirror ? e + 26 - 2 * (e % 27) : e)];
     if (v[i] >= n_in) v[i] = -1;
   }
   float xv[NI][CIN];
@@ -283,6 +285,8 @@
   __shared__ int idxS[NW_ROWS * 27];
   __shared__ int maskS[NW_ROWS];
   const int t = threadIdx.x, co = t & 63, wv = t >> 6;
+  const int mirror = accumulate & 2;
+  accumulate &= 1;
   float w[27][CIN];
 #pragma unroll
   for (int k = 0; k < 27; ++k)
@@ -292,7 +296,7 @@
   const int tiles = (n_out + NW_ROWS - 1) / NW_ROWS;
   for (int tile = blockIdx.x; tile < tiles; tile += gridDim.x) {
     const int row0 = tile * NW_ROWS;
-    narrow_stage<CIN>(X, ldx, nbr, row0, n_out, n_in, xg, idxS, maskS);
+    narrow_stage<CIN>(X, ldx, nbr, row0, n_out, n_in, xg, idxS, maskS, mirror);
     for (int rr = 0; rr < NW_ROWS / 4; ++rr) {
       const int r = wv * (NW_ROWS / 4) + rr;
       if (row0 + r >= n_out) break;
@@ -320,6 +324,7 @@
                              void* stream) {
   if (n_out <= 0 || Cout <= 0) return 0;
   if (K > MAXK) return -2;
+  if ((accumulate & 2) && (!(K & 1) || nbr == nullptr)) return -3;
   if (!trans_w && narrow_ok(nbr, K, Cin, Cout)) {
     const int tiles = es_cdiv(n_out, NW_ROWS);
     hipLaunchKernelGGL(k_spconv_narrow_fwd<3>, dim3(tiles > 2048 ? 2048 : tiles), dim3(256), 0, (hipStream_t)stream, X, ldx, W, nbr,
@@ -598,6 +603,7 @@
 
 #define ES_IO_Y16 1
 #define ES_IO_R16 2
+#define ES_IO_MIRROR 0x20000
 #define ES_IO_WSHARE 0x10000
 __device__ __forceinline__ float4 bf16x4_to_f32(uint2 v) {
   return make_float4(__uint_as_float(v.x << 16), __uint_as_float(v.x & 0xffff0000u), __uint_as_float(v.y << 16),
@@ -630,6 +636,7 @@
   __shared__ int tapAny[32];
   const int t = threadIdx.x, lane = t & 63, wv = t >> 6;
   const int row0 = blockIdx.x * BM, n0 = blockIdx.y * BNT;
+  const int mirror = io & ES_IO_MIRROR;
   const bool vecA = ((ldx & 3) == 0) && ((((uintptr_t)X) & 15) == 0);
   const bool vecB = ((Cin & 7) == 0) && ((((uintptr_t)W) & 15) == 0);
 
@@ -638,7 +645,7 @@
   for (int e = t; e < BM * K; e += 256) {
     int r = e / K, k = e - r * K;
     int j = row0 + r, v = -1;
-    if (j < n_out) v = nbr ? nbr[(size_t)j * K + k] : (j < n_in ? j : -1);
+    if (j < n_out) v = nbr ? nbr[(size_t)j * K + (mirror ? K - 1 - k : k)] : (j < n_in ? j : -1);
     nbrS[e] = v;
     if (v >= 0) tapAny[k] = 1;
   }
@@ -875,7 +882,7 @@
     const int* src = nbr ? nbr + (size_t)j * K : nullptr;
     for (int k = k0; k < k1; ++k) {
       int v = -1;
-      if (j < n_out) v = src ? src[k] : (j < n_in ? j : -1);
+      if (j < n_out) v = src ? src[(io & ES_IO_MIRROR) ? K - 1 - k : k] : (j < n_in ? j : -1);
       nbrS[r * K + k] = v;
       if (v >= 0) tapFlag[k] = 1;
     }
@@ -1108,7 +1115,7 @@
     const int* src = nbr ? nbr + (size_t)j * K : nullptr;
     for (int k = k0; k < k1; ++k) {
       int v = -1;
-      if (j < n_out) v = src ? src[k] : (j < n_in ? j : -1);
+      if (j < n_out) v = src ? src[(io & ES_IO_MIRROR) ? K - 1 - k : k] : (j < n_in ? j : -1);
       nbrS[r * K + k] = v;
       if (v >= 0) tapFlag[k] = 1;
     }
@@ -1799,7 +1806,10 @@
                                 int y_half = 0, int r_half = 0) {
   if (n_out <= 0 || Cout <= 0) return 0;
   if (K > MAXK) return -2;
-  int io = (y_half ? ES_IO_Y16 : 0) | ((r_half && ep_res) ? ES_IO_R16 : 0) | (y_half & 0xff00);
+  const int mirror = accumulate & 2;
+  accumulate &= 1;
+  if (mirror && (!(K & 1) || nbr == nullptr)) return -3;
+  int io = (mirror ? ES_IO_MIRROR : 0) | (y_half ? ES_IO_Y16 : 0) | ((r_half && ep_res) ? ES_IO_R16 : 0) | (y_half & 0xff00);
   if (y_half && (accumulate || (ldy % 4) || (Cout % 4) || (((uintptr_t)Y) & 7))) return -7;
   if ((io & ES_IO_R16) && ((ep_ldr % 4) || (((uintptr_t)ep_res) & 7))) return -7;
   hipStream_t st = (hipStream_t)stream;
diff --git a/embodiedscan_amd/engine.py b/embodiedscan_amd/engine.py
--- a/embodiedscan_amd/engine.py
+++ b/embodiedscan_amd/engine.py
@@ -471,6 +471,12 @@
 HALO = [os.environ.get('ES_HALO', '1') != '0']
 if os.environ.get('ES_HALO_MIN_WGS') is not None:
     hip.raw('es_halo_set_option')(30, int(os.environ['ES_HALO_MIN_WGS']))
+if os.environ.get('ES_HALO_PLAN_BITMAP') is not None:
+    hip.raw('es_halo_set_option')(32, int(os.environ['ES_HALO_PLAN_BITMAP']))
+
+
+def _is_mirror(inv):
+    return inv is not None and not isinstance(inv, torch.Tensor)
 
 
 def _halo_ok(nbr, n_out, n_in, ldx, K, cin, cout):
@@ -494,7 +500,7 @@
 
 
 def _halo_launch(Xh, ldx, Wp, nbr, n_out, n_in, K, cin, cout, bias_p, Y, ldy, acc):
-    fwd = getattr(nbr, '_mirror_of', None)
+    fwd = nbr.nbr if _is_mirror(nbr) else getattr(nbr, '_mirror_of', None)
     loc, hrows, hcnt = halo_plan(fwd if fwd is not None else nbr)
     return hip.try_call('es_spconv_halo_bf16', Xh, ldx, Wp, P(loc), P(hrows), P(hcnt), n_out, n_in, K, cin, cout, bias_p, Y, ldy, acc,
                         int(fwd is not None), _stream())
@@ -702,6 +708,8 @@
                 and hip.try_call('es_img_dgrad3_s2_bf16', P(gy), _ld(gy), P(w.bf16()[0]), img[0], img[1], img[2], cin, P(gate), P(x.d),
                                  _ld(x.d), P(x.g), _ld(x.g), s)):
             return
+        if _is_mirror(inv):
+            inv = inv.real()
         if x.d.dtype == torch.bfloat16:
             call('es_spconv_fwd_bf16_io', P(gy), 0, _ld(gy), P(w.bf16()[0]), P(inv), n_in, n_out, K, cout, cin, P(gate), 0,
                  P(x.d), 1, _ld(x.d), 3, P(x.g), 0, _ld(x.g), s)
@@ -723,6 +731,8 @@
     if gh is not None and _halo_ok(inv, n_in, n_out, cout, K, cout, cin) and \
             _halo_launch(P(gh), cout, P(w.bf16()[0]), inv, n_in, n_out, K, cout, cin, 0, P(g), _ld(g), acc):
         return
+    if _is_mirror(inv):
+        inv, acc = inv.nbr, acc | 2
     if gh is not None:
         _fwd_bf16(P(gh), 1, cout, P(w.bf16()[0]), P(inv), n_in, n_out, K, cout, cin, 0, P(g), _ld(g), acc, gh)
     elif bf and cout >= 16:
diff --git a/embodiedscan_amd/hip.py b/embodiedscan_amd/hip.py
--- a/embodiedscan_amd/hip.py
+++ b/embodiedscan_amd/hip.py
@@ -55,6 +55,8 @@
                   (16, 'ES_SPLIT_FOLD'), (19, 'ES_RG128_MIN_WGS'), (20, 'ES_WSHARE'), (21, 'ES_NARROW'), (23, 'ES_RG320'), (24, 'ES_LIN_SMALL'), (25, 'ES_EXPAND'), (26, 'ES_EXPAND_WGS')):
     if os.environ.get(_env) is not None:
         _fn['es_set_option'](_key, int(os.environ[_env]))
+if os.environ.get('ES_FOCAL_INFLIGHT') is not None:
+    _fn['es_losses_set_option'](40, int(os.environ['ES_FOCAL_INFLIGHT']))
 
 
 class HipError(RuntimeError):
diff --git a/embodiedscan_amd/models/backbones/mink_resnet.py b/embodiedscan_amd/models/backbones/mink_resnet.py
--- a/embodiedscan_amd/models/backbones/mink_resnet.py
+++ b/embodiedscan_amd/models/backbones/mink_resnet.py
@@ -60,7 +60,7 @@
                 cs.inverse_map(oc, k)
             cs = oc
             cs.kernel_map(cs, 3)
-            cs.inverse_map(cs, 3)
+            cs.self_inverse(3)
 
     def forward(self, x):
         tr = self.training
@@ -84,12 +84,12 @@
                     idt = blk['down'][1](idt, act=0, training=tr)
                     cs = oc
                 else:
-                    o = E.conv(f, blk['conv1'], cs.kernel_map(cs, 3), cs.inverse_map(cs, 3), cs.n)
+                    o = E.conv(f, blk['conv1'], cs.kernel_map(cs, 3), cs.self_inverse(3), cs.n)
                     idt = f
                 c1 = o
                 o = blk['norm1'](o, act=1, training=tr)
                 n1 = o
-                o = E.conv(o, blk['conv2'], cs.kernel_map(cs, 3), cs.inverse_map(cs, 3), cs.n)
+                o = E.conv(o, blk['conv2'], cs.kernel_map(cs, 3), cs.self_inverse(3), cs.n)
                 f = blk['norm2'](o, act=1, res=idt, training=tr)
                 if self.trace is not None:
                     self.trace += [c1, n1, o, f]
diff --git a/embodiedscan_amd/models/dense_heads/fcaf3d_head.py b/embodiedscan_amd/models/dense_heads/fcaf3d_head.py
--- a/embodiedscan_amd/models/dense_heads/fcaf3d_head.py
+++ b/embodiedscan_amd/models/dense_heads/fcaf3d_head.py
@@ -86,7 +86,7 @@
 
 def conv3(st, w, out_set=None):
     cs = st.cs
-    nbr, inv = cs.kernel_map(cs, 3), cs.inverse_map(cs, 3)
+    nbr, inv = cs.kernel_map(cs, 3), cs.self_inverse(3)
     return SparseTensor(cs, E.conv(st.F, w, nbr, inv, cs.n))
 
 
@@ -160,17 +160,17 @@
         x = level_sets[-1]
         thr = self.pts_prune_threshold
         if maps:
-            x.kernel_map(x, 3), x.inverse_map(x, 3)
+            x.kernel_map(x, 3), x.self_inverse(3)
         for i in range(len(level_sets) - 2, -1, -1):
             c = x.children()
             if maps:
-                c.kernel_map(c, 3), c.inverse_map(c, 3)
+                c.kernel_map(c, 3), c.self_inverse(3)
             u, _, _ = sparse.union(c, level_sets[i])
             off = u.offsets()
             if any(off[b + 1] - off[b] > thr for b in range(u.n_batch)):
                 break
             if maps:
-                u.kernel_map(u, 3), u.inverse_map(u, 3)
+                u.kernel_map(u, 3), u.self_inverse(3)
             x = u
 
     def _levels(self, inputs):
diff --git a/embodiedscan_amd/models/necks/mink_neck.py b/embodiedscan_amd/models/necks/mink_neck.py
--- a/embodiedscan_amd/models/necks/mink_neck.py
+++ b/embodiedscan_amd/models/necks/mink_neck.py
@@ -49,17 +49,17 @@
         x = level_sets[-1]
         thr = self.pts_prune_threshold
         if maps:
-            x.kernel_map(x, 3), x.inverse_map(x, 3)
+            x.kernel_map(x, 3), x.self_inverse(3)
         for i in range(len(level_sets) - 2, -1, -1):
             c = x.children()
             if maps:
-                c.kernel_map(c, 3), c.inverse_map(c, 3)
+                c.kernel_map(c, 3), c.self_inverse(3)
             u, _, _ = sparse.union(c, level_sets[i])
             off = u.offsets()
             if any(off[b + 1] - off[b] > thr for b in range(u.n_batch)):
                 break
             if maps:
-                u.kernel_map(u, 3), u.inverse_map(u, 3)
+                u.kernel_map(u, 3), u.self_inverse(3)
             x = u
 
     def levels(self, inputs):
diff --git a/embodiedscan_amd/sparse.py b/embodiedscan_amd/sparse.py
--- a/embodiedscan_amd/sparse.py
+++ b/embodiedscan_amd/sparse.py
@@ -1,4 +1,5 @@
 import ctypes
+import os
 import weakref
 
 import torch
@@ -115,12 +116,30 @@
             self.cache[key] = (hip.register_map(inv), weakref.ref(out))
         return inv
 
+    def self_inverse(self, ksize):
+        if MIRROR_TAPS[0] and ksize % 2 == 1:
+            return MirrorInv(self, ksize, self.kernel_map(self, ksize))
+        return self.inverse_map(self, ksize)
+
     def children(self):
         if 'gen' not in self.cache:
             keys = torch.empty(self.n * 8, dtype=torch.int64, device=self.device)
             call('es_gen_children_keys', P(self.keys), self.n, self.ts // 2, P(keys), _stream())
             self.cache['gen'] = CoordSet(keys, self.n * 8, self.ts // 2, self.n_batch)
         return self.cache['gen']
+
+
+MIRROR_TAPS = [os.environ.get('ES_MIRROR_TAPS', '1') != '0']
+
+
+class MirrorInv:
+    __slots__ = ('cs', 'ksize', 'nbr')
+
+    def __init__(self, cs, ksize, nbr):
+        self.cs, self.ksize, self.nbr = cs, ksize, nbr
+
+    def real(self):
+        return self.cs.inverse_map(self.cs, self.ksize)
 
 
 COORD_BATCH = [__import__('os').environ.get('ES_COORD_BATCH', '1') != '0']
diff --git a/include/es_hip.h b/include/es_hip.h
--- a/include/es_hip.h
+++ b/include/es_hip.h
@@ -158,6 +158,7 @@
 int es_focal_loss_clear(const float* logits, int ldl, const int* labels, int N, int C, float gamma, float alpha,
                         const float* avg_factor_dev, float grad_scale, float* grad, int ldg, double* partial ,
                         float* loss_out , int lead, int tail, void* stream);
+int es_losses_set_option(int key, int value);
 int es_reg_decode_fwd(const float* reg, int ldr, int n, const float* scale, float* bbox , void* stream);
 int es_reg_decode_bwd(const float* reg, int ldr, const float* bbox, const float* dbbox, int n, const float* scale,
                       float* dreg, int ldg, float* dscale, float* partial, void* stream);
```
